# lqhl/rabitq-rs

Measured on AMD Instinct MI355X. Metric: queries/sec at recall@10>=0.95, GIST-1M d=960, batch=1024, higher is better.
Workload: dtype u8

## Files before the change

### include/rbq.h

```cpp
#ifndef RBQ_H
#define RBQ_H

#include <stddef.h>
#include <stdint.h>

#ifdef __cplusplus
extern "C" {
#endif

#define RBQ_OK                   0
#define RBQ_DIMENSION_MISMATCH   1
#define RBQ_INVALID_CONFIG       2
#define RBQ_EMPTY_INDEX          3
#define RBQ_IO                   4
#define RBQ_INVALID_PERSISTENCE  5
#define RBQ_DEVICE               6

#define RBQ_METRIC_L2 0
#define RBQ_METRIC_IP 1
#define RBQ_ROTATOR_MATRIX 0
#define RBQ_ROTATOR_FHT_KAC 1
#define RBQ_ROTATOR_NONE 2

#define RBQ_BATCH 32

typedef struct rbq_index rbq_index;
typedef struct rbq_builder rbq_builder;

typedef struct {
    uint32_t dim;
    uint32_t padded_dim;
    uint8_t  metric;
    uint8_t  rotator;
    uint8_t  ex_bits;
    uint8_t  reserved;
    uint64_t n_vectors;
    uint64_t n_lists;
    const uint8_t* rotator_blob;
    uint64_t rotator_len;
} rbq_header;

typedef struct {
    const float*    centroid;
    uint64_t        n;
    const uint64_t* ids;
    const uint8_t*  batch_data;
    uint64_t        batch_len;
    const uint8_t*  ex_codes;
    const float*    f_add_ex;
    const float*    f_rescale_ex;
} rbq_list_view;

typedef struct {
    uint64_t estimated;
    uint64_t skipped_by_lower_bound;
    uint64_t extended_evaluations;
} rbq_diag;

int rbq_index_create(const rbq_header* hdr, const rbq_list_view* lists,
                     int n_devices, const int* devices, rbq_index** out);

int rbq_index_load_rbq1(const void* bytes, size_t len,
                        int n_devices, const int* devices, rbq_index** out);

int rbq_index_build_device(const rbq_header* hdr, const float* centroids, const float* d_data, const uint32_t* d_assign,
                           uint64_t n, float t_const, int device, rbq_index** out);

#define RBQ_RESCALE_CONST   0
#define RBQ_RESCALE_OPTIMAL 1
int rbq_index_build_device_ex(const rbq_header* hdr, const float* centroids, const float* d_data, const uint32_t* d_assign,
                              uint64_t n, int rescale, float t_const, int device, rbq_index** out);

int rbq_build_stream_begin(const rbq_header* hdr, const float* centroids, const uint32_t* list_sizes, float t_const,
                           int device, rbq_builder** out);
int rbq_build_stream_begin_ex(const rbq_header* hdr, const float* centroids, const uint32_t* list_sizes, int rescale,
                              float t_const, int device, rbq_builder** out);
int rbq_build_stream_push(rbq_builder* b, const float* vectors, const uint32_t* assign, uint64_t first_id, uint64_t count);
int rbq_build_stream_finish(rbq_builder* b, int n_devices, const int* devices, rbq_index** out);
void rbq_build_stream_abort(rbq_builder* b);

void rbq_index_destroy(rbq_index* idx);

uint64_t rbq_index_len(const rbq_index* idx);
uint64_t rbq_index_cluster_count(const rbq_index* idx);
uint32_t rbq_index_dim(const rbq_index* idx);
uint32_t rbq_index_padded_dim(const rbq_index* idx);
uint32_t rbq_index_device_count(const rbq_index* idx);

int rbq_search_batch(const rbq_index* idx, const float* queries, uint64_t nq,
                     uint32_t query_dim, uint32_t top_k, uint32_t nprobe,
                     const uint32_t* filter_words, uint64_t filter_nbits,
                     uint64_t* out_ids, float* out_scores, uint32_t* out_counts,
                     rbq_diag* diag);

int rbq_posting_scan_batch(const rbq_index* idx, const float* queries, uint64_t nq, uint32_t query_dim,
                           uint32_t top_k, const uint32_t* list_ids, const uint32_t* list_counts,
                           uint32_t max_lists, uint64_t* out_ids, float* out_scores, uint32_t* out_counts);



int rbq_search_batch_device(const rbq_index* idx, const float* d_queries, uint64_t nq,
                            uint32_t query_dim, uint32_t top_k, uint32_t nprobe,
                            const uint32_t* d_filter_words, uint64_t filter_nbits,
                            uint64_t* d_out_ids, float* d_out_scores,
                            uint32_t* d_out_counts, rbq_diag* d_diag,
                            void* hip_stream);

int rbq_release_stream(rbq_index* idx, void* hip_stream);

int rbq_index_fetch_embeddings(const rbq_index* idx, const uint64_t* ids, uint64_t n, float* out, uint8_t* found);
int rbq_index_fetch_embeddings_device(const rbq_index* idx, const uint64_t* d_ids, uint64_t n, float* d_out,
                                      uint8_t* d_found, void* hip_stream);

void* rbq_host_alloc(size_t bytes);
void rbq_host_free(void* p);

int rbq_index_set_rerank_vectors(rbq_index* idx, const float* vectors, uint64_t n);

#define RBQ_NUMERIC_NATIVE_AVX512 0
#define RBQ_NUMERIC_NATIVE_AVX2   1
#define RBQ_NUMERIC_PORTABLE      2
int rbq_index_set_numeric_variant(rbq_index* idx, int variant);
int rbq_index_numeric_variant(const rbq_index* idx);

void   rbq_profile_begin(rbq_index* idx);
void   rbq_profile_end(rbq_index* idx);
double rbq_profile_stage_ms(const rbq_index* idx, const char* stage, uint64_t* launches);
uint64_t rbq_profile_stage_samples(const rbq_index* idx, const char* stage, float* out, uint64_t cap);
uint64_t rbq_profile_scan_bytes(const rbq_index* idx);
int rbq_profile_counters(const rbq_index* idx, uint64_t* out, uint32_t n);
void rbq_profile_select_stages(rbq_index* idx, uint32_t mask);
void rbq_profile_set_sampling(rbq_index* idx, uint32_t every);
uint64_t rbq_debug_rank_fallbacks(const rbq_index* idx);
void rbq_debug_tie_log_stats(const rbq_index* idx, uint64_t* out4);
int rbq_debug_stage_resources(rbq_index* idx, uint64_t nq, uint32_t top_k, uint32_t nprobe, uint32_t* out);
uint64_t rbq_debug_bounce_copies(void);
uint64_t rbq_debug_head_exact_evaluations(const rbq_index* idx);
uint64_t rbq_debug_head_exact_guard_trips(const rbq_index* idx);
uint64_t rbq_debug_heap_restarts(const rbq_index* idx);
int rbq_debug_copy_index(rbq_index* idx, const char* name, void* dst, uint64_t bytes);
int rbq_debug_best_rescale(const float* o_abs, uint64_t n, uint32_t dim, uint32_t ex_bits, int device, double* out_t);
int rbq_debug_copy_workspace(rbq_index* idx, void* hip_stream, const char* name, void* dst, uint64_t bytes);
int rbq_debug_set_option(rbq_index* idx, const char* name, int value);

int rbq_process_defaults(void);
const char* rbq_strerror(int code);
int rbq_last_error_detail(char* buf, size_t n);

uint32_t rbq_abi_version(void);

#ifdef __cplusplus
}
#endif

#include "rbq_bf.h"
#include "rbq_kmeans.h"
#include "rbq_persist.h"

#endif
```

### rabitq-rs_amd/csrc/device/api.hpp

```cpp
#pragma once
#include <hip/hip_runtime.h>

#include <algorithm>
#include <atomic>
#include <chrono>
#include <condition_variable>
#include <deque>
#include <functional>
#include <cmath>
#include <cstdio>
#include <cstdlib>
#include <cstring>
#include <map>
#include <memory>
#include <mutex>
#include <new>
#include <string>
#include <thread>
#include <vector>

#include "rbq.h"
#include "launch.hpp"
#include "../host/rbq_host_logic.hpp"

// ... 123 lines not shown
        if (e == hipSuccess) events.push_back(*ev);
        return e;
    }
};

template <class Job, int kThreads>
struct WorkerPool {
    std::thread th[kThreads];
    std::mutex mu;
    std::condition_variable cv;
    std::deque<Job> jobs;
    std::atomic<uint32_t> pending{0};
    bool stop = false;
    void run() {
        for (;;) {
            Job job;
            {
                std::unique_lock<std::mutex> lk(mu);
                cv.wait(lk, [this] { return stop || !jobs.empty(); });
                if (jobs.empty()) return;
                job = std::move(jobs.front());
                jobs.pop_front();
            }
            job();
            pending.fetch_sub(1, std::memory_order_release);
            (void)spin_until([this] { return pending.load(std::memory_order_acquire) != 0; }, std::chrono::microseconds(100));
        }
    }
    bool start() {
        try {
            for (auto& t : th) t = std::thread([this] { run(); });
        } catch (...) {
            shutdown();
            return false;
        }
        return true;
    }
    void post(Job j) {
        pending.fetch_add(1, std::memory_order_release);
        { std::lock_guard<std::mutex> lk(mu); jobs.push_back(std::move(j)); }
        cv.notify_one();
    }
    void shutdown() {
        { std::lock_guard<std::mutex> lk(mu); stop = true; }
        cv.notify_all();
        for (auto& t : th) if (t.joinable()) t.join();
    }
};

struct StageJob {
    void* dst = nullptr;
    const void* src = nullptr;
    size_t bytes = 0;
    std::atomic<int>* done = nullptr;
    void operator()() const {
        std::memcpy(dst, src, bytes);
        done->store(1, std::memory_order_release);
    }
};
using StagePool = WorkerPool<StageJob, 3>;

using ReplicaPool = WorkerPool<std::function<void()>, 2>;

struct Workspace {
    hipStream_t stream = nullptr;
    DevBuf queries, rot, lut, consts, scores, probe, wl, nstream, nvec, out_pack, filter, rot_hi, rot_lo, dead_skipped, heap_ws, key_window, audit_dead, tie_log, head_ub;
    DevBuf ms_sl, ms_lists;
    DevBuf mr_pool;
    PinBuf h_in, h_out;
    hipEvent_t done = nullptr;
    uint64_t call_nq = 0;
    bool latency_first = false;
    Workspace() = default;
    Workspace(const Workspace&) = delete;
    ~Workspace() {
        if (done) (void)hipEventDestroy(done);
        if (stream) (void)hipStreamDestroy(stream);
    }
};

struct StageProf {
    std::vector<std::pair<hipEvent_t, hipEvent_t>> ev;
    double ms = 0;
    uint64_t launches = 0;
    std::vector<float> samples;
};
struct EventPool {
    std::vector<std::pair<hipEvent_t, hipEvent_t>> free_pairs;
    bool take(std::pair<hipEvent_t, hipEvent_t>& p) {
        if (!free_pairs.empty()) { p = free_pairs.back(); free_pairs.pop_back(); return true; }
        if (hipEventCreateWithFlags(&p.first, hipEventDisableSystemFence) != hipSuccess) return false;
        if (hipEventCreateWithFlags(&p.second, hipEventDisableSystemFence) != hipSuccess) { (void)hipEventDestroy(p.first); return false; }
        return true;
    }
    void give(const std::pair<hipEvent_t, hipEvent_t>& p) { free_pairs.push_back(p); }
    void destroy() {
        for (auto& e : free_pairs) { (void)hipEventDestroy(e.first); (void)hipEventDestroy(e.second); }
        free_pairs.clear();
    }
};

struct Arr {
    void* p = nullptr;
    size_t bytes = 0;
};

struct Geometry {
    uint32_t dim = 0, D = 0, Dc = 0;
    uint8_t metric = 0, rotator = 0, ex_bits = 0;
    uint32_t trunc = 0;
    float fac = 1.0f;
};
inline Geometry geometry_of(const rbq_header& h) {
    Geometry g;
    g.dim = h.dim; g.D = h.padded_dim; g.Dc = (h.padded_dim + 63u) / 64u * 64u;
    g.metric = h.metric; g.rotator = h.rotator; g.ex_bits = h.ex_bits;
    uint32_t lg = 0;
    for (uint32_t x = h.dim; x >>= 1;) ++lg;
    g.trunc = 1u << lg;
    g.fac = 1.0f / std::sqrt((float)g.trunc);
    return g;
}

template <class Ws>
PrepParams prep_params(const Geometry& g, const Arr& rot_blob, Ws& w, const float* queries, uint64_t nq) {
    PrepParams p;
    p.queries = queries; p.nq = (uint32_t)nq; p.dim = g.dim; p.D = g.D; p.Dc = g.Dc; p.rotator = (int)g.rotator;
    p.rot_blob = (const uint8_t*)rot_blob.p; p.trunc = g.trunc; p.fac = g.fac; p.ex_bits = g.ex_bits;
    p.rot = (float*)w.rot.p; p.lut = (uint8_t*)w.lut.p; p.consts = (QueryConsts*)w.consts.p;
    p.rot_hi = nullptr; p.rot_lo = nullptr; p.wg_prep = false;
    return p;
}

inline int scan_wave_default() {
    static const int v = [] { const char* e = std::getenv("RBQ_SCAN_WAVE"); return e && *e ? std::atoi(e) : 2; }();
    return v;
}

struct Options {
    uint32_t numeric_variant = 0;
    uint32_t host_lanes = 0, host_subbatch = 0, host_trace = 0;
    int rank_ksplit = 1;
    bool host_zero_copy = true;
    bool host_stage_helpers = true;
    bool no_block_bound = false, f32_rank = false, wg_prep = false, exact_heap = false, force_rank_fallback = false, exact_rank = false;
    bool head_exact = true;
    bool lazy_filter = true;
    bool lazy_fault_inject = false;
    SlackMul slack;
    int slack_term = 0;
    bool ub_tap = false;
    bool lazy_audit = false;
    bool lazy_select = true;
    uint32_t tie_log_cap = 0;
    bool tie_log = true;
    int latency_path = 1;
    int rank_tile = 0;
    uint32_t stage_mask = 0xf;
    int scan_wave = scan_wave_default();
    bool profile_counters = true;
    uint64_t save_chunk = 0;
    uint64_t fetch_chunk = 0;
    uint64_t mstg_chunk = 0;
    uint64_t mstg_search_budget = 0;
    int set(const char* name, int value);
};

struct Replica : Geometry {
    int device = 0;
    uint64_t n_vectors = 0, n_lists = 0, n_blocks = 0;
    Arr rot_blob, centroids, blocks, ids, ex, fadd_ex, fres_ex, list_gb0, list_n, prof, bsum, cnorm2, fallbacks, cent_hi, cent_lo, raw,
        bsumx, lsum;
    Arr* arrays[18] = {&rot_blob, &centroids, &blocks, &ids, &ex, &fadd_ex, &fres_ex, &list_gb0, &list_n, &prof, &bsum, &cnorm2,
                       &fallbacks, &cent_hi, &cent_lo, &raw, &bsumx, &lsum};
    Arr delta, vl;
    Arr rnorm;
    bool has_rnorm = false, tc_some = false;
    float tc_value = 0.0f;
    bool has_recon = false;
    std::mutex fetch_mu;
    Arr fmap_ids, fmap_slots;
    bool fmap_ready = false;
    Arr ms_hi, ms_lo, ms_nc;
    bool ms_ready = false;
    uint32_t ms_bad = 0;
    Arr mr_slot_map, mr_blk_list;
    bool mr_ready = false;
    float cnorm2_max = 0.0f;
    uint64_t n_raw = 0;
    bool raw_borrowed = false;
    bool rerank = false;
    Options opt;
    std::unique_ptr<StagePool> stagers;
    bool stagers_failed = false;
    std::vector<uint32_t> h_list_n;
    std::vector<uint64_t> nblk_desc_prefix;
    std::mutex mu;
    std::vector<Workspace*> pool;
    std::map<hipStream_t, Workspace*> stream_ws;
    bool profiling = false;
    uint32_t prof_mask = 0xf;
    uint32_t prof_every = 1;
    uint32_t prof_seq[4] = {0, 0, 0, 0};
    StageProf stage_prof[4];
    EventPool ev_pool;
    uint64_t prof_counters[kProfSlots] = {0, 0, 0, 0, 0, 0, 0, 0};
    Replica() = default;
    Replica(const Replica&) = delete;
};

int alloc_arr(Arr& a, size_t bytes);
int upload_arr(Arr& a, const void* src, size_t bytes);
void free_replica(Replica* ix);
struct ReplicaOwner {
    Replica* ix;
    ~ReplicaOwner() { if (ix) free_replica(ix); }
    Replica* release() { Replica* r = ix; ix = nullptr; return r; }
};
int validate_header(const rbq_header* h, bool brute_force = false);
int resolve_devices(int n_devices, const int* devices, std::vector<int>& out);
Replica* new_replica(const rbq_header* hdr, int dev);
int finish_replica(Replica* ix, const std::vector<uint32_t>& ln);
int wrap_and_replicate(Replica* first, const std::vector<int>& devs, rbq_index** out);
int build_device_pairs(const rbq_header* hdr, const float* centroids, const float* d_data, const uint32_t* d_assign,
                       const uint32_t* d_vec, uint64_t n, int rescale, float t_const, int dev, rbq_index** out);

Workspace* take_ws(Replica* ix);
void give_ws(Replica* ix, Workspace* w);
Workspace* stream_workspace(Replica* ix, hipStream_t s);
int check_query_args(const rbq_index* h, uint32_t query_dim);
Replica* replica_of_pointer(rbq_index* h, const void* dptr);
struct ProfScope {
    Replica* ix; int stage; hipStream_t s; std::pair<hipEvent_t, hipEvent_t> ev{nullptr, nullptr};
    bool on = false, ext = false;
    ProfScope(Replica* ix_, int st, hipStream_t s_, bool ext_ = false) : ix(ix_), stage(st), s(s_), ext(ext_) {
        if (ix->profiling && !stage_probes() && ((ix->prof_mask >> st) & 1u)) {
            {
                std::lock_guard<std::mutex> g(ix->mu);
                if (ix->prof_seq[st]++ % ix->prof_every == 0) on = ix->ev_pool.take(ev);
            }
            if (on && !ext) (void)hipEventRecord(ev.first, s);
        }
    }
    hipEvent_t start() const { return on && ext ? ev.first : nullptr; }
    hipEvent_t stop() const { return on && ext ? ev.second : nullptr; }
    ~ProfScope() {
        if (on) {
            if (!ext) (void)hipEventRecord(ev.second, s);
            std::lock_guard<std::mutex> g(ix->mu);
            ix->stage_prof[stage].ev.push_back(ev);
        }
    }
};
int scan_stage(Replica* ix, Workspace* w, uint64_t nq, uint32_t probe_stride, uint32_t top_k, uint64_t wl_stride,
               const uint32_t* d_filter, uint64_t filter_nbits, uint64_t* d_ids, float* d_scores, uint32_t* d_counts,
               rbq_diag* d_diag, bool mstg, const uint32_t* d_dead_skipped, hipStream_t stream, const uint64_t* d_slot_ids = nullptr);

}

struct rbq_index {
    std::vector<rbq_api::Replica*> reps;
    int debug_replica = 0;
    std::mutex worker_mu;
    std::vector<std::unique_ptr<rbq_api::ReplicaPool>> workers;
};

#pragma GCC visibility pop
```

### rabitq-rs_amd/csrc/device/api_index.hip

```cpp
#include "api.hpp"

using namespace rbq_api;

extern "C" int rbq_process_defaults(void) {
    return RBQ_OK;
}

namespace rbq_api {
int alloc_arr(Arr& a, size_t bytes) {
    HIP_TRY(hipMalloc(&a.p, bytes ? bytes : 16));
    a.bytes = bytes;
    return RBQ_OK;
}
int upload_arr(Arr& a, const void* src, size_t bytes) {
    int rc = alloc_arr(a, bytes);
    if (rc) return rc;
    if (bytes) HIP_TRY(hipMemcpy(a.p, src, bytes, hipMemcpyHostToDevice));
    return RBQ_OK;
}

void free_replica(Replica* ix) {
    if (!ix) return;
    if (ix->stagers) ix->stagers->shutdown();
    DeviceGuard g(ix->device);
    (void)hipDeviceSynchronize();
    for (Arr* a : ix->arrays)
        if (a->p && !(a == &ix->raw && ix->raw_borrowed)) (void)hipFree(a->p);
    for (Arr* a : {&ix->delta, &ix->vl, &ix->rnorm, &ix->fmap_ids, &ix->fmap_slots, &ix->ms_hi, &ix->ms_lo, &ix->ms_nc,
                   &ix->mr_slot_map, &ix->mr_blk_list})
        if (a->p) (void)hipFree(a->p);
    for (Workspace* w : ix->pool) delete w;
    for (auto& kv : ix->stream_ws) delete kv.second;
    for (auto& sp : ix->stage_prof)
        for (auto& e : sp.ev) { (void)hipEventDestroy(e.first); (void)hipEventDestroy(e.second); }
    ix->ev_pool.destroy();
    delete ix;
}

int validate_header(const rbq_header* h, bool brute_force) {
    if (!h) return fail(RBQ_INVALID_CONFIG, "null header");
    if (h->dim == 0) return fail(RBQ_INVALID_CONFIG, "dimension must be positive");
    if (h->padded_dim < h->dim) return fail(RBQ_INVALID_CONFIG, "padded_dim must be >= dim");
    if (h->metric > 1) return fail(RBQ_INVALID_CONFIG, "unknown metric tag");
    if (h->rotator > (brute_force ? RBQ_ROTATOR_FHT_KAC : RBQ_ROTATOR_NONE)) return fail(RBQ_INVALID_CONFIG, "unknown rotator type tag");
    if (h->ex_bits != 0 && h->ex_bits != 2 && h->ex_bits != 6)
        return fail(RBQ_INVALID_CONFIG, "Unsupported ex_bits: only 0 (1-bit total), 2 (3-bit total), and 6 (7-bit total) are supported");
    if (h->padded_dim % 16 != 0) return fail(RBQ_INVALID_CONFIG, "Dimension must be multiple of 16 for SIMD");
    if (h->padded_dim > 2048)
        return fail(RBQ_INVALID_CONFIG, "padded_dim > 2048 (high-accuracy i32 LUT mode) is not supported");
    if (h->rotator_len != 0 && !h->rotator_blob) return fail(RBQ_INVALID_CONFIG, "null rotator blob");
    if (h->rotator == RBQ_ROTATOR_NONE) {
        if (h->padded_dim != h->dim) return fail(RBQ_INVALID_CONFIG, "rotator NONE requires padded_dim == dim");
        if (h->rotator_len != 0) return fail(RBQ_INVALID_CONFIG, "rotator NONE takes no rotator blob");
    } else if (h->rotator == RBQ_ROTATOR_FHT_KAC) {
        if (h->padded_dim % 64 != 0) return fail(RBQ_INVALID_CONFIG, "FHT rotator requires dimension to be multiple of 64");
        if (h->rotator_len != (uint64_t)4 * h->padded_dim / 8) return fail(RBQ_INVALID_PERSISTENCE, "FHT rotator flip bits length mismatch");
    } else {
        if (h->rotator_len != (uint64_t)h->padded_dim * h->padded_dim * 4) return fail(RBQ_INVALID_PERSISTENCE, "rotator matrix length mismatch");
    }
    if (brute_force) return RBQ_OK;
    if (h->n_lists == 0) return fail(RBQ_INVALID_CONFIG, "nlist must be positive");
    if (h->n_lists > 0xffffffffull) return fail(RBQ_INVALID_CONFIG, "too many lists");
    return RBQ_OK;
}

int resolve_devices(int n_devices, const int* devices, std::vector<int>& out) {
    if (n_devices < 1 || n_devices > 16) return fail(RBQ_INVALID_CONFIG, "n_devices must be in 1..16");
    int count = 0;
    HIP_TRY(hipGetDeviceCount(&count));
    out.clear();
    for (int i = 0; i < n_devices; ++i) {
        int d = 0;
        if (devices) d = devices[i];
        else if (n_devices == 1) HIP_TRY(hipGetDevice(&d));
        else d = i;
        if (d < 0 || d >= count) return fail(RBQ_INVALID_CONFIG, "no such device: " + std::to_string(d));
        out.push_back(d);
    }
    return RBQ_OK;
}

Replica* new_replica(const rbq_header* hdr, int dev) {
    Replica* ix = new Replica();
    static_cast<Geometry&>(*ix) = geometry_of(*hdr);
    ix->device = dev;
    ix->n_lists = hdr->n_lists;
    return ix;
}

int finish_replica(Replica* ix, const std::vector<uint32_t>& ln) {
    const uint32_t nlist = (uint32_t)ix->n_lists, D = ix->D;
    ix->h_list_n = ln;
    {
        std::vector<uint64_t> nblk(nlist);
        for (uint32_t c = 0; c < nlist; ++c) nblk[c] = (ln[c] + 31u) / 32u;
        std::sort(nblk.begin(), nblk.end(), std::greater<uint64_t>());
        ix->nblk_desc_prefix.assign((size_t)nlist + 1, 0);
        for (uint32_t c = 0; c < nlist; ++c) ix->nblk_desc_prefix[c + 1] = ix->nblk_desc_prefix[c] + nblk[c];
    }
    int rc;
    if ((rc = alloc_arr(ix->cnorm2, (size_t)nlist * 4))) return rc;
    if ((rc = alloc_arr(ix->cent_hi, (size_t)nlist * D * 2))) return rc;
    if ((rc = alloc_arr(ix->cent_lo, (size_t)nlist * D * 2))) return rc;
    HIP_TRY(launch_centroid_arrays((const float*)ix->centroids.p, nlist, D, (float*)ix->cnorm2.p, (uint16_t*)ix->cent_hi.p,
                                   (uint16_t*)ix->cent_lo.p, 0));
    std::vector<float> cn(nlist);
    HIP_TRY(hipMemcpy(cn.data(), ix->cnorm2.p, (size_t)nlist * 4, hipMemcpyDeviceToHost));
    double mx = 0;
    for (float v : cn) if (std::isfinite(v)) mx = std::max(mx, (double)v);
    ix->cnorm2_max = (float)(mx * 1.000001);
    if ((rc = alloc_arr(ix->lsum, (size_t)nlist * sizeof(BlockSummary)))) return rc;
    if ((rc = alloc_arr(ix->bsumx, ix->n_blocks * sizeof(BlockSummaryEx)))) return rc;
    HIP_TRY(launch_list_summaries((const uint8_t*)ix->blocks.p, (const uint8_t*)ix->ex.p, (const float*)ix->fadd_ex.p,
                                  (const float*)ix->fres_ex.p, (const float*)ix->centroids.p, (const BlockSummary*)ix->bsum.p,
                                  (const uint32_t*)ix->list_gb0.p, (const uint32_t*)ix->list_n.p, nlist, D, ix->Dc, ix->ex_bits,
                                  (BlockSummaryEx*)ix->bsumx.p, (BlockSummary*)ix->lsum.p, 0));
    if ((rc = alloc_arr(ix->fallbacks, 32))) return rc;
    HIP_TRY(hipMemset(ix->fallbacks.p, 0, 32));
    if ((rc = alloc_arr(ix->prof, (size_t)kProfStripes * kProfSlots * 8))) return rc;
    HIP_TRY(hipMemset(ix->prof.p, 0, (size_t)kProfStripes * kProfSlots * 8));
    const char* e = std::getenv("RBQ_EXACT_RANK");
    ix->opt.exact_rank = e && e[0] == '1';
    const char* f = std::getenv("RBQ_FORCE_RANK_FALLBACK");
    ix->opt.force_rank_fallback = f && f[0] == '1';
    const char* lz = std::getenv("RBQ_LAZY_SELECT");
    ix->opt.lazy_select = !(lz && lz[0] == '0');
    return RBQ_OK;
}

int Options::set(const char* name, int v) {
    const auto is = [name](const char* n) { return !std::strcmp(name, n); };
    if (is("block_bound")) no_block_bound = v == 0;
    else if (is("exact_rank")) exact_rank = v != 0;
    else if (is("exact_heap")) exact_heap = v != 0;
    else if (is("lazy_select")) lazy_select = v != 0;
    else if (is("rank_tile")) rank_tile = v;
    else if (is("latency_path")) latency_path = v;
    else if (is("tie_log")) tie_log = v != 0;
    else if (is("tie_log_cap")) tie_log_cap = v > 0 ? (uint32_t)v : 0u;
    else if (is("stage_mask")) stage_mask = (uint32_t)v & 0xfu;
    else if (is("scan_wave")) scan_wave = v < 0 ? scan_wave_default() : (v > 2 ? 2 : v);
    else if (is("profile_counters")) profile_counters = v != 0;
    else if (is("f32_rank")) f32_rank = v != 0;
    else if (is("wg_prep")) wg_prep = v != 0;
    else if (is("force_rank_fallback")) force_rank_fallback = v != 0;
    else if (is("host_lanes")) host_lanes = v > 0 ? (uint32_t)v : 0u;
    else if (is("host_subbatch")) host_subbatch = v > 0 ? (uint32_t)v : 0u;
    else if (is("host_trace")) host_trace = v != 0;
    else if (is("lazy_fault_inject")) lazy_fault_inject = v != 0;
    else if (is("lazy_audit")) lazy_audit = v != 0;
    else if (is("ub_tap")) ub_tap = v != 0;
    else if (is("save_chunk")) save_chunk = v > 0 ? (uint64_t)v : 0u;
    else if (is("fetch_chunk")) fetch_chunk = v > 0 ? (uint64_t)v : 0u;
    else if (is("mstg_chunk")) mstg_chunk = v > 0 ? (uint64_t)v : 0u;
    else if (is("mstg_search_budget")) mstg_search_budget = v > 0 ? (uint64_t)v : 0u;
    else if (is("slack_term")) slack_term = v;
    else if (is("slack_milli")) {
        float* f[6] = {&slack.ge, &slack.eip, &slack.est, &slack.lb, &slack.et, &slack.dist};
        if (slack_term < 0 || slack_term > 5) return fail(RBQ_INVALID_CONFIG, "slack_term is 0..5");
        *f[slack_term] = (float)v * 1e-3f;
    }
    else if (is("head_exact")) head_exact = v != 0;
    else if (is("lazy_filter")) lazy_filter = v != 0;
    else if (is("host_zero_copy")) host_zero_copy = v != 0;
    else if (is("rank_ksplit")) rank_ksplit = v < 0 ? 0 : v;
    else if (is("host_stage_helpers")) host_stage_helpers = v != 0;
    else return fail(RBQ_INVALID_CONFIG, std::string("unknown option ") + name);
    return RBQ_OK;
}
}

namespace rbq_api {
namespace {
void free_index(rbq_index* h) {
    if (!h) return;
    for (auto& w : h->workers) w->shutdown();
    for (Replica* r : h->reps) free_replica(r);
    delete h;
}

std::atomic<uint64_t> g_bounce_copies{0};
hipError_t copy_cross_device(void* dst, int ddev, const void* src, int sdev, size_t bytes) {
    if (!bytes) return hipSuccess;
    const char* fnp = std::getenv("RBQ_FORCE_NO_PEER");
    const bool no_peer = fnp && fnp[0] == '1';
    hipError_t e = hipSuccess;
    if (!no_peer) {
        if (ddev == sdev) return hipMemcpy(dst, src, bytes, hipMemcpyDeviceToDevice);
        int can = 0;
        if (hipDeviceCanAccessPeer(&can, ddev, sdev) == hipSuccess && can) {
            const hipError_t pe = hipDeviceEnablePeerAccess(sdev, 0);
            if (pe != hipSuccess) (void)hipGetLastError();
        } else {
            (void)hipGetLastError();
        }
        e = hipMemcpyPeer(dst, ddev, src, sdev, bytes);
        if (e == hipSuccess) return e;
        (void)hipGetLastError();
    }
    g_bounce_copies.fetch_add(1, std::memory_order_relaxed);
    const size_t CH = (size_t)64 << 20;
    void* bounce = nullptr;
    e = hipHostMalloc(&bounce, std::min(bytes, CH), hipHostMallocPortable);
    if (e != hipSuccess) return e;
    for (size_t off = 0; off < bytes && e == hipSuccess; off += CH) {
        const size_t n = std::min(CH, bytes - off);
        e = hipSetDevice(sdev);
        if (e == hipSuccess) e = hipMemcpy(bounce, (const uint8_t*)src + off, n, hipMemcpyDeviceToHost);
        if (e == hipSuccess) e = hipSetDevice(ddev);
        if (e == hipSuccess) e = hipMemcpy((uint8_t*)dst + off, bounce, n, hipMemcpyHostToDevice);
    }
    (void)hipSetDevice(ddev);
    (void)hipHostFree(bounce);
    return e;
}

int clone_replica(const Replica* src, int dev, Replica** out) {
    DeviceGuard g(dev);
    if (!g.ok) return fail(RBQ_DEVICE, "hipSetDevice failed");
    Replica* ix = new Replica();
    static_cast<Geometry&>(*ix) = *src;
    ix->device = dev;
    ix->n_vectors = src->n_vectors; ix->n_lists = src->n_lists; ix->n_blocks = src->n_blocks;
    ix->cnorm2_max = src->cnorm2_max; ix->h_list_n = src->h_list_n; ix->nblk_desc_prefix = src->nblk_desc_prefix;
    ix->opt = src->opt;
    for (size_t i = 0; i < sizeof(ix->arrays) / sizeof(ix->arrays[0]); ++i) {
        const Arr* s = src->arrays[i];
        Arr* d = ix->arrays[i];
        if (!s->p || s == &src->raw) continue;
        hipError_t e = hipMalloc(&d->p, s->bytes ? s->bytes : 16);
        if (e == hipSuccess && s->bytes) e = copy_cross_device(d->p, dev, s->p, src->device, s->bytes);
        if (e != hipSuccess) { free_replica(ix); return fail(RBQ_DEVICE, std::string("replicating the index: ") + hipGetErrorString(e)); }
        d->bytes = s->bytes;
    }
    hipError_t e = hipMemset(ix->fallbacks.p, 0, 32);
    if (e == hipSuccess) e = hipMemset(ix->prof.p, 0, (size_t)kProfStripes * kProfSlots * 8);
    if (e != hipSuccess) { free_replica(ix); return fail(RBQ_DEVICE, hipGetErrorString(e)); }
    *out = ix;
    return RBQ_OK;
}
}

int wrap_and_replicate(Replica* first, const std::vector<int>& devs, rbq_index** out) {
    rbq_index* h = new rbq_index();
    h->reps.push_back(first);
    for (size_t i = 1; i < devs.size(); ++i) {
        Replica* r = nullptr;
        int rc = clone_replica(first, devs[i], &r);
        if (rc) { free_index(h); return rc; }
        h->reps.push_back(r);
    }
    *out = h;
    return RBQ_OK;
}

namespace {
int create_from_sources(const rbq_header* hdr, const std::vector<ListSrc>& lists, int dev, Replica** out) {
    DeviceGuard g(dev);
    if (!g.ok) return fail(RBQ_DEVICE, "hipSetDevice failed");
    ReplicaOwner own{new_replica(hdr, dev)};
    Replica* ix = own.ix;
    Scratch cl;
    const uint32_t D = ix->D, Dc = ix->Dc, nlist = (uint32_t)ix->n_lists, exbits = ix->ex_bits;
    const size_t ref_stride = (size_t)D * 4 + 384, dev_stride = (size_t)Dc * 4 + 384, exb = (size_t)D * exbits / 8;
    const size_t exd = ex_bytes_dev(D, exbits);
    std::vector<uint32_t> gb0(nlist), ln(nlist);
    uint64_t nblocks = 0, nvec = 0;
    bool recon = true;
    for (uint32_t c = 0; c < nlist; ++c)
        if (lists[c].n && (!lists[c].delta || !lists[c].vl)) recon = false;
    for (uint32_t c = 0; c < nlist; ++c) {
        const ListSrc& L = lists[c];
        if (L.n > 0xffffffffull) return fail(RBQ_INVALID_CONFIG, "list too large");
        gb0[c] = (uint32_t)nblocks; ln[c] = (uint32_t)L.n;
        nblocks += (L.n + 31) / 32; nvec += L.n;
        if (nblocks * 32 > 0xffffffffull) return fail(RBQ_INVALID_CONFIG, "index too large for 32-bit vector slots");
    }
    ix->n_blocks = nblocks; ix->n_vectors = nvec;
    const uint64_t nslots = nblocks * 32;
    int rc;
    if ((rc = upload_arr(ix->rot_blob, hdr->rotator_blob, hdr->rotator_len))) return rc;
    if ((rc = upload_arr(ix->list_gb0, gb0.data(), (size_t)nlist * 4))) return rc;
    if ((rc = upload_arr(ix->list_n, ln.data(), (size_t)nlist * 4))) return rc;
    {
        std::vector<float> cent((size_t)nlist * D);
        for (uint32_t c = 0; c < nlist; ++c) std::memcpy(&cent[(size_t)c * D], lists[c].centroid, (size_t)D * 4);
        if ((rc = upload_arr(ix->centroids, cent.data(), cent.size() * 4))) return rc;
    }
    if ((rc = alloc_arr(ix->blocks, nblocks * dev_stride))) return rc;
    if ((rc = alloc_arr(ix->ids, nslots * 8))) return rc;
    if ((rc = alloc_arr(ix->ex, exd ? nslots * exd + 256 : 0))) return rc;
    if ((rc = alloc_arr(ix->fadd_ex, exbits ? nslots * 4 : 0))) return rc;
    if ((rc = alloc_arr(ix->fres_ex, exbits ? nslots * 4 : 0))) return rc;
    if ((rc = alloc_arr(ix->bsum, nblocks * sizeof(BlockSummary)))) return rc;
    if (recon) {
        if ((rc = alloc_arr(ix->delta, nslots * 4))) return rc;
        if ((rc = alloc_arr(ix->vl, nslots * 4))) return rc;
    }

    const size_t per_block = ref_stride + 32 * (exb + 24) + 12 + 64;
    uint64_t chunk_blocks = std::max<uint64_t>(1, ((size_t)64 << 20) / per_block);
    chunk_blocks = std::min<uint64_t>(chunk_blocks, std::max<uint64_t>(nblocks, 1));
    const size_t cap = align_up(chunk_blocks * ref_stride, 16) + align_up(chunk_blocks * 32 * exb, 16) + chunk_blocks * 32 * 24 +
                       chunk_blocks * 12 + 256;
    uint8_t* pin[2] = {nullptr, nullptr};
    uint8_t* dst[2] = {nullptr, nullptr};
    hipEvent_t ev[2] = {nullptr, nullptr};
    HIP_TRY(cl.make_stream());
    for (int i = 0; i < 2; ++i) {
        HIP_TRY(cl.alloc_pinned(&pin[i], cap));
        HIP_TRY(cl.alloc(&dst[i], cap));
        HIP_TRY(cl.event(&ev[i]));
    }
    uint32_t c = 0;
    uint64_t lb = 0;
    uint64_t b0 = 0;
    int turn = 0;
    while (b0 < nblocks) {
        const uint64_t nb = std::min<uint64_t>(chunk_blocks, nblocks - b0);
        const int i = turn & 1;
        if (turn >= 2) HIP_TRY(hipEventSynchronize(ev[i]));
        uint8_t* base = pin[i];
        const size_t o_recs = 0, o_ex = align_up(nb * ref_stride, 16);
        const size_t o_ids = o_ex + align_up(nb * 32 * exb, 16), o_fadd = o_ids + nb * 32 * 8, o_fres = o_fadd + nb * 32 * 4,
                     o_dl = o_fres + nb * 32 * 4, o_vl = o_dl + nb * 32 * 4, o_d0 = o_vl + nb * 32 * 4, o_nv = o_d0 + nb * 8,
                     total = o_nv + nb * 4;
        uint64_t* dense0 = reinterpret_cast<uint64_t*>(base + o_d0);
        uint32_t* nvb = reinterpret_cast<uint32_t*>(base + o_nv);
        uint64_t filled = 0, dense = 0;
        while (filled < nb) {
            while (c < nlist && lb >= ((uint64_t)ln[c] + 31) / 32) { ++c; lb = 0; }
            const ListSrc& L = lists[c];
            const uint64_t lnb = ((uint64_t)ln[c] + 31) / 32, take = std::min<uint64_t>(lnb - lb, nb - filled);
            const uint64_t v0 = lb * 32, v1 = std::min<uint64_t>(L.n, (lb + take) * 32), nv = v1 - v0;
            std::memcpy(base + o_recs + filled * ref_stride, L.batch_data + lb * ref_stride, take * ref_stride);
            if (nv) std::memcpy(base + o_ids + dense * 8, L.ids + v0 * 8, nv * 8);
            if (exbits && nv) {
                if (L.ex_stride == exb) std::memcpy(base + o_ex + dense * exb, L.ex + v0 * exb, nv * exb);
                else for (uint64_t v = 0; v < nv; ++v) std::memcpy(base + o_ex + (dense + v) * exb, L.ex + (v0 + v) * L.ex_stride, exb);
                std::memcpy(base + o_fadd + dense * 4, L.fadd + v0 * 4, nv * 4);
                std::memcpy(base + o_fres + dense * 4, L.fres + v0 * 4, nv * 4);
            }
            if (recon && nv) {
                std::memcpy(base + o_dl + dense * 4, L.delta + v0 * 4, nv * 4);
                std::memcpy(base + o_vl + dense * 4, L.vl + v0 * 4, nv * 4);
            }
            for (uint64_t b = 0; b < take; ++b) {
                dense0[filled + b] = dense + b * 32;
                nvb[filled + b] = (uint32_t)std::min<uint64_t>(32, L.n - (lb + b) * 32);
            }
            filled += take; dense += nv; lb += take;
        }
        uint8_t* d = dst[i];
        HIP_TRY(hipMemcpyAsync(d, base, total, hipMemcpyHostToDevice, cl.stream));
        const uint64_t* d_d0 = reinterpret_cast<const uint64_t*>(d + o_d0);
        const uint32_t* d_nv = reinterpret_cast<const uint32_t*>(d + o_nv);
        uint8_t* oblocks = (uint8_t*)ix->blocks.p + b0 * dev_stride;
        HIP_TRY(launch_relayout_blocks(d + o_recs, (uint32_t)nb, D, Dc, oblocks, cl.stream));
        HIP_TRY(launch_block_summary(oblocks, d_nv, (uint32_t)nb, Dc, (BlockSummary*)ix->bsum.p + b0, cl.stream));
        HIP_TRY(launch_spread_u64(reinterpret_cast<const uint64_t*>(d + o_ids), d_d0, d_nv, (uint32_t)nb, ~0ull,
                                  (uint64_t*)ix->ids.p + b0 * 32, cl.stream));
        if (exbits) {
            HIP_TRY(launch_relayout_ex(d + o_ex, d_d0, d_nv, (uint32_t)nb, D, exbits, (uint8_t*)ix->ex.p + b0 * 32 * exd, cl.stream));
            HIP_TRY(launch_spread_f32(reinterpret_cast<const float*>(d + o_fadd), d_d0, d_nv, (uint32_t)nb, 0.0f,
                                      (float*)ix->fadd_ex.p + b0 * 32, cl.stream));
            HIP_TRY(launch_spread_f32(reinterpret_cast<const float*>(d + o_fres), d_d0, d_nv, (uint32_t)nb, 0.0f,
                                      (float*)ix->fres_ex.p + b0 * 32, cl.stream));
        }
        if (recon) {
            HIP_TRY(launch_spread_f32(reinterpret_cast<const float*>(d + o_dl), d_d0, d_nv, (uint32_t)nb, 0.0f,
                                      (float*)ix->delta.p + b0 * 32, cl.stream));
            HIP_TRY(launch_spread_f32(reinterpret_cast<const float*>(d + o_vl), d_d0, d_nv, (uint32_t)nb, 0.0f,
                                      (float*)ix->vl.p + b0 * 32, cl.stream));
        }
        HIP_TRY(hipEventRecord(ev[i], cl.stream));
        b0 += nb;
        ++turn;
    }
    if (exd) HIP_TRY(hipMemsetAsync((uint8_t*)ix->ex.p + nslots * exd, 0, 256, cl.stream));
    HIP_TRY(hipStreamSynchronize(cl.stream));
    if ((rc = finish_replica(ix, ln))) return rc;
    HIP_TRY(hipDeviceSynchronize());
    ix->has_recon = recon;
    *out = own.release();
    return RBQ_OK;
}

int create_impl(const rbq_header* hdr, const rbq_list_view* lists, const float* const* delta, const float* const* vl, int n_devices,
// ... 137 lines not shown
                if (e != hipSuccess) rc = fail(RBQ_DEVICE, std::string("attaching the rerank vectors: ") + hipGetErrorString(e));
            }
        }
        if (rc != RBQ_OK) {
            const std::string keep = g_err;
            for (size_t r = 0; r < R; ++r)
                if (fresh[r].p && !borrowed[r]) { DeviceGuard g(h->reps[r]->device); (void)hipFree(fresh[r].p); }
            return fail(rc, keep);
        }
    }
    for (size_t r = 0; r < R; ++r) {
        Replica* ix = h->reps[r];
        DeviceGuard g(ix->device);
        if (!g.ok) return fail(RBQ_DEVICE, "hipSetDevice failed");
        HIP_TRY(hipDeviceSynchronize());
        if (ix->raw.p && !ix->raw_borrowed) (void)hipFree(ix->raw.p);
        ix->raw = Arr(); ix->n_raw = 0; ix->rerank = false; ix->raw_borrowed = false;
        if (!attach) continue;
        ix->raw = fresh[r]; ix->raw_borrowed = borrowed[r] != 0;
        ix->n_raw = n; ix->rerank = true;
    }
    return RBQ_OK;
    RBQ_GUARD_END
}

void* rbq_host_alloc(size_t bytes) {
    void* p = nullptr;
    if (hipHostMalloc(&p, bytes ? bytes : 16, hipHostMallocPortable) != hipSuccess) { (void)hipGetLastError(); return nullptr; }
    return p;
}
void rbq_host_free(void* p) { if (p) (void)hipHostFree(p); }

void rbq_profile_begin(rbq_index* h) {
    if (!h) return;
    for (Replica* ix : h->reps) {
        DeviceGuard g(ix->device);
        std::lock_guard<std::mutex> lk(ix->mu);
        for (auto& sp : ix->stage_prof) {
            for (auto& e : sp.ev) ix->ev_pool.give(e);
            sp.ev.clear(); sp.ms = 0; sp.launches = 0; sp.samples.clear();
        }
        for (auto& c : ix->prof_counters) c = 0;
        (void)hipMemset(ix->prof.p, 0, (size_t)kProfStripes * kProfSlots * 8);
        ix->profiling = true;
    }
}
void rbq_profile_end(rbq_index* h) {
    if (!h) return;
    for (Replica* ix : h->reps) {
        DeviceGuard g(ix->device);
        (void)hipDeviceSynchronize();
        std::lock_guard<std::mutex> lk(ix->mu);
        ix->profiling = false;
        std::vector<unsigned long long> c((size_t)kProfStripes * kProfSlots, 0ull);
        (void)hipMemcpy(c.data(), ix->prof.p, c.size() * 8, hipMemcpyDeviceToHost);
        for (int i = 0; i < kProfSlots; ++i) {
            ix->prof_counters[i] = 0;
            for (uint32_t st = 0; st < kProfStripes; ++st) ix->prof_counters[i] += c[(size_t)st * kProfSlots + i];
        }
        for (auto& sp : ix->stage_prof) {
            for (auto& e : sp.ev) {
                float ms = 0;
                if (hipEventElapsedTime(&ms, e.first, e.second) == hipSuccess) { sp.ms += ms; sp.launches++; sp.samples.push_back(ms); }
                ix->ev_pool.give(e);
            }
            sp.ev.clear();
        }
    }
}
double rbq_profile_stage_ms(const rbq_index* h, const char* stage, uint64_t* launches) {
    if (!h || h->reps.empty() || !stage) return -1;
    int s = !std::strcmp(stage, "prep") ? 0 : !std::strcmp(stage, "rank") ? 1 : !std::strcmp(stage, "select") ? 2 : !std::strcmp(stage, "scan") ? 3 : -1;
    if (s < 0) return -1;
    double ms = 0; uint64_t n = 0;
    for (const Replica* ix : h->reps) { ms += ix->stage_prof[s].ms; n += ix->stage_prof[s].launches; }
    if (launches) *launches = n;
    return n ? ms / (double)n : 0.0;
}
uint64_t rbq_profile_stage_samples(const rbq_index* h, const char* stage, float* out, uint64_t cap) {
    if (!h || h->reps.empty() || !stage) return 0;
    int s = !std::strcmp(stage, "prep") ? 0 : !std::strcmp(stage, "rank") ? 1 : !std::strcmp(stage, "select") ? 2 : !std::strcmp(stage, "scan") ? 3 : -1;
    if (s < 0) return 0;
    uint64_t n = 0;
    for (const Replica* ix : h->reps)
        for (float v : ix->stage_prof[s].samples) { if (out && n < cap) out[n] = v; ++n; }
    return n;
}
uint64_t rbq_profile_scan_bytes(const rbq_index* h) {
    if (!h || h->reps.empty()) return 0;
    uint64_t v = 0;
    for (const Replica* ix : h->reps) v += ix->prof_counters[kProfVectorsProbed];
    return v * (uint64_t)(h->reps[0]->D / 8 + 12);
}
int rbq_profile_counters(const rbq_index* h, uint64_t* out, uint32_t n) {
    if (!h || h->reps.empty() || !out) return RBQ_INVALID_CONFIG;
    for (uint32_t i = 0; i < n; ++i) {
        out[i] = 0;
        if (i < (uint32_t)kProfSlots) for (const Replica* ix : h->reps) out[i] += ix->prof_counters[i];
    }
    return RBQ_OK;
}
void rbq_profile_select_stages(rbq_index* h, uint32_t mask) { if (h) for (Replica* ix : h->reps) ix->prof_mask = mask & 0xfu; }
void rbq_profile_set_sampling(rbq_index* h, uint32_t every) { if (h) for (Replica* ix : h->reps) ix->prof_every = every ? every : 1u; }

int rbq_index_set_numeric_variant(rbq_index* h, int variant) {
    g_err.clear();
    if (!h || h->reps.empty()) return fail(RBQ_INVALID_CONFIG, "null index");
    if (variant != RBQ_NUMERIC_NATIVE_AVX512 && variant != RBQ_NUMERIC_NATIVE_AVX2 && variant != RBQ_NUMERIC_PORTABLE)
        return fail(RBQ_INVALID_CONFIG, "numeric variant " + std::to_string(variant) +
                                            " is not one of 0 (native_avx512), 1 (native_avx2), 2 (portable)");
    static_assert(RBQ_NUMERIC_NATIVE_AVX512 == kVarAvx512 && RBQ_NUMERIC_NATIVE_AVX2 == kVarAvx2 && RBQ_NUMERIC_PORTABLE == kVarPortable,
                  "the ABI values are the kernels' variant numbers");
    for (Replica* ix : h->reps) ix->opt.numeric_variant = (uint32_t)variant;
    return RBQ_OK;
}
int rbq_index_numeric_variant(const rbq_index* h) {
    if (!h || h->reps.empty()) return -1;
    return (int)h->reps[0]->opt.numeric_variant;
}

int rbq_debug_set_option(rbq_index* h, const char* name, int value) {
    if (!h || h->reps.empty() || !name) return RBQ_INVALID_CONFIG;
    if (!std::strcmp(name, "numeric_variant")) return rbq_index_set_numeric_variant(h, value);
    if (!std::strcmp(name, "debug_replica")) {
        if (value < 0 || (size_t)value >= h->reps.size()) return fail(RBQ_INVALID_CONFIG, "no such replica");
        h->debug_replica = value;
        return RBQ_OK;
    }
    for (Replica* ix : h->reps) {
        int rc;
        if (!std::strcmp(name, "rerank")) {
            if (value && !ix->raw.p) return fail(RBQ_INVALID_CONFIG, "no raw vectors attached (rbq_index_set_rerank_vectors)");
            ix->rerank = value != 0;
        } else if ((rc = ix->opt.set(name, value))) {
            return rc;
        }
    }
    return RBQ_OK;
}
static uint64_t read_counter(const rbq_index* h, int slot) {
    if (!h) return 0;
    uint64_t tot = 0;
    for (const Replica* ix : h->reps) {
        unsigned int v = 0;
        DeviceGuard g(ix->device);
        (void)hipDeviceSynchronize();
        (void)hipMemcpy(&v, (const unsigned int*)ix->fallbacks.p + slot, 4, hipMemcpyDeviceToHost);
        tot += v;
    }
    return tot;
}
uint64_t rbq_debug_rank_fallbacks(const rbq_index* h) { return read_counter(h, 0); }
void rbq_debug_tie_log_stats(const rbq_index* h, uint64_t* out4) { if (out4) for (int i = 0; i < 4; ++i) out4[i] = read_counter(h, 4 + i); }
uint64_t rbq_debug_head_exact_guard_trips(const rbq_index* h) { return read_counter(h, 2); }
uint64_t rbq_debug_head_exact_evaluations(const rbq_index* h) { return read_counter(h, 3); }


uint64_t rbq_debug_bounce_copies(void) { return g_bounce_copies.load(std::memory_order_relaxed); }
uint64_t rbq_debug_heap_restarts(const rbq_index* h) { return read_counter(h, 1); }


int rbq_debug_copy_workspace(rbq_index* h, void* hip_stream, const char* name, void* dst, uint64_t bytes) {
    g_err.clear();
    RBQ_GUARD_BEGIN
    if (!h || h->reps.empty() || !name || !dst) return RBQ_INVALID_CONFIG;
    Replica* ix = h->reps[h->debug_replica];
    Workspace* w = nullptr;
    {
        std::lock_guard<std::mutex> lk(ix->mu);
        auto it = ix->stream_ws.find((hipStream_t)hip_stream);
        if (it != ix->stream_ws.end()) w = it->second;
    }
    if (!w) return fail(RBQ_INVALID_CONFIG, "no workspace for this stream");
    static const std::pair<const char*, DevBuf Workspace::*> kBufs[] = {
        {"rot", &Workspace::rot}, {"lut", &Workspace::lut}, {"consts", &Workspace::consts}, {"scores", &Workspace::scores},
        {"probe", &Workspace::probe}, {"nstream", &Workspace::nstream}, {"wl", &Workspace::wl}, {"nvec", &Workspace::nvec},
        {"dead_skipped", &Workspace::dead_skipped}, {"audit_dead", &Workspace::audit_dead}, {"head_ub", &Workspace::head_ub},
        {"rot_hi", &Workspace::rot_hi}, {"rot_lo", &Workspace::rot_lo}};
    DevBuf* b = nullptr;
    for (const auto& kb : kBufs) if (!std::strcmp(name, kb.first)) b = &(w->*kb.second);
    if (!b || !b->p || bytes > b->cap) return fail(RBQ_INVALID_CONFIG, "unknown buffer or size");
    DeviceGuard g(ix->device);
    HIP_TRY(hipMemcpy(dst, b->p, bytes, hipMemcpyDeviceToHost));
    return RBQ_OK;
    RBQ_GUARD_END
}

int rbq_debug_copy_index(rbq_index* h, const char* name, void* dst, uint64_t bytes) {
    g_err.clear();
    RBQ_GUARD_BEGIN
    if (!h || h->reps.empty() || !name || !dst) return RBQ_INVALID_CONFIG;
    Replica* ix = h->reps[h->debug_replica];
    const size_t stride = (size_t)ix->Dc * 4 + 384, exd = ex_bytes_dev(ix->D, ix->ex_bits), slots = ix->n_blocks * 32;
    const void* p = nullptr;
    size_t have = 0;
    if (!std::strcmp(name, "blocks")) { p = ix->blocks.p; have = ix->n_blocks * stride; }
    else if (!std::strcmp(name, "ids")) { p = ix->ids.p; have = slots * 8; }
    else if (!std::strcmp(name, "ex")) { p = ix->ex.p; have = slots * exd; }
    else if (!std::strcmp(name, "fadd_ex")) { p = ix->fadd_ex.p; have = ix->ex_bits ? slots * 4 : 0; }
    else if (!std::strcmp(name, "fres_ex")) { p = ix->fres_ex.p; have = ix->ex_bits ? slots * 4 : 0; }
    else if (!std::strcmp(name, "bsum")) { p = ix->bsum.p; have = ix->n_blocks * sizeof(BlockSummary); }
    else if (!std::strcmp(name, "lsum")) { p = ix->lsum.p; have = ix->n_lists * sizeof(BlockSummary); }
    else if (!std::strcmp(name, "bsumx")) { p = ix->bsumx.p; have = ix->n_blocks * sizeof(BlockSummaryEx); }
    else if (!std::strcmp(name, "centroids")) { p = ix->centroids.p; have = ix->n_lists * ix->D * 4; }
    else if (!std::strcmp(name, "list_gb0")) { p = ix->list_gb0.p; have = ix->n_lists * 4; }
    else if (!std::strcmp(name, "list_n")) { p = ix->list_n.p; have = ix->n_lists * 4; }
    else if (!std::strcmp(name, "cent_hi")) { p = ix->cent_hi.p; have = ix->n_lists * ix->D * 2; }
    else if (!std::strcmp(name, "cent_lo")) { p = ix->cent_lo.p; have = ix->n_lists * ix->D * 2; }
    else if (!std::strcmp(name, "cnorm2")) { p = ix->cnorm2.p; have = ix->n_lists * 4; }
    else if (!std::strcmp(name, "delta") || !std::strcmp(name, "vl")) {
        ix = h->reps[0];
        p = name[0] == 'd' ? ix->delta.p : ix->vl.p; have = ix->has_recon ? ix->n_blocks * 32 * 4 : 0;
    }
    else if (!std::strcmp(name, "rnorm")) {
        ix = h->reps[0];
        p = ix->rnorm.p; have = ix->has_rnorm ? ix->n_blocks * 32 * 4 : 0;
    }
    if (!p || bytes != have) return fail(RBQ_INVALID_CONFIG, "unknown array or size (have " + std::to_string(have) + " bytes)");
    DeviceGuard g(ix->device);
    HIP_TRY(hipMemcpy(dst, p, bytes, hipMemcpyDeviceToHost));
    return RBQ_OK;
    RBQ_GUARD_END
}
}
```

### rabitq-rs_amd/csrc/device/api_search.hip

```cpp
#include "api.hpp"

using namespace rbq_api;

namespace rbq_api {
namespace {
constexpr uint64_t kScanWaveMinQueries = 128;
constexpr uint64_t kHostWaveMinQueries = 4096;
constexpr uint64_t kLatMaxQueries = 4;
constexpr uint64_t kLatMaxBytes = 96ull << 20;
constexpr uint64_t kSplitKMaxCallQueries = 256;
constexpr uint64_t kPrepWgMaxQueries = 512;
constexpr uint64_t kZeroCopyMinQueries = 5;


bool is_pinned_host_range(const void* p, size_t bytes) {
    if (!p) return false;
    hipPointerAttribute_t a, b;
    if (hipPointerGetAttributes(&a, p) != hipSuccess) { (void)hipGetLastError(); return false; }
    if (a.type != hipMemoryTypeHost) return false;
    if (bytes <= 1) return true;
    const uint8_t* last = (const uint8_t*)p + bytes - 1;
    if (hipPointerGetAttributes(&b, last) != hipSuccess) { (void)hipGetLastError(); return false; }
    if (b.type != hipMemoryTypeHost) return false;
    if (a.devicePointer && b.devicePointer && (const uint8_t*)b.devicePointer - (const uint8_t*)a.devicePointer != (ptrdiff_t)(bytes - 1)) return false;
// ... 42 lines not shown
    if (hipPointerGetAttributes(&a, dptr) == hipSuccess) {
        for (Replica* r : h->reps) if (r->device == a.device) return r;
    } else {
        (void)hipGetLastError();
    }
    return h->reps[0];
}

int scan_stage(Replica* ix, Workspace* w, uint64_t nq, uint32_t probe_stride, uint32_t top_k, uint64_t wl_stride,
               const uint32_t* d_filter, uint64_t filter_nbits, uint64_t* d_ids, float* d_scores, uint32_t* d_counts,
               rbq_diag* d_diag, bool mstg, const uint32_t* d_dead_skipped, hipStream_t stream, const uint64_t* d_slot_ids) {
    ProfScope ps(ix, 3, stream, true);
    ScanParams P;
    P.blocks = (const uint8_t*)ix->blocks.p; P.ids = d_slot_ids ? d_slot_ids : (const uint64_t*)ix->ids.p; P.ex_codes = (const uint8_t*)ix->ex.p;
    P.f_add_ex = (const float*)ix->fadd_ex.p; P.f_rescale_ex = (const float*)ix->fres_ex.p;
    P.lut = (const uint8_t*)w->lut.p; P.rot = (const float*)w->rot.p; P.consts = (const QueryConsts*)w->consts.p;
    P.probe = (const ProbeInfo*)w->probe.p; P.wl = (const StreamItem*)w->wl.p; P.nstream = (const uint32_t*)w->nstream.p;
    P.filter = d_filter; P.filter_nbits = filter_nbits; P.wl_stride = wl_stride;
    P.out_ids = d_ids; P.out_scores = d_scores; P.out_counts = d_counts; P.diag = (unsigned long long*)d_diag;
    P.D = ix->D; P.Dc = ix->Dc; P.nprobe = probe_stride; P.top_k = top_k; P.metric = ix->metric;
    P.ex_bits = mstg ? 0u : ix->ex_bits;
    P.no_block_bound = ix->opt.no_block_bound ? 1u : 0u;
    P.exact_heap = ix->opt.exact_heap ? 1u : 0u;
    P.heap_restarts = (unsigned int*)ix->fallbacks.p + 1;
    P.tie_stats = (unsigned int*)ix->fallbacks.p + 4;
    P.mstg = mstg ? 1u : 0u;
    P.prof = (ix->profiling && ix->opt.profile_counters) ? (unsigned long long*)ix->prof.p : nullptr;
    P.dead_skipped = d_dead_skipped;
    P.numeric_variant = ix->opt.numeric_variant;
    P.wave_kernel = (ix->opt.scan_wave == 1 || (ix->opt.scan_wave == 2 && nq >= kScanWaveMinQueries && !ix->opt.no_block_bound && !w->latency_first)) ? 1u : 0u;
    P.tie_log = nullptr; P.tie_log_cap = 0;
    if (ix->opt.tie_log && !P.wave_kernel && !d_diag && !mstg && top_k >= 1 && top_k <= kTopKRegMax && !ix->opt.exact_heap && !stage_probes()) {
        const uint32_t cap = ix->opt.tie_log_cap ? ix->opt.tie_log_cap : (top_k < 64u ? 2048u : 8192u);
        if ((uint64_t)nq * cap * 12u <= (1ull << 30)) {
            if (w->tie_log.ensure((size_t)nq * cap * 12u) == RBQ_OK) { P.tie_log = (uint32_t*)w->tie_log.p; P.tie_log_cap = cap; }
            else { (void)hipGetLastError(); g_err.clear(); }
        }
    }
    P.heap_ws = nullptr;
    if (top_k > kTopKMax || scan_lds_bytes(ix->Dc, ix->D, P.ex_bits, top_k) > kLdsPerWorkgroupMax) {
        int rc = w->heap_ws.ensure((size_t)nq * 2 * ((size_t)top_k + 1) * 4);
        if (rc) return rc;
        P.heap_ws = (uint32_t*)w->heap_ws.p;
    }
    HIP_TRY(launch_scan(P, (uint32_t)nq, ix->device, stream, ps.start(), ps.stop()));
    return RBQ_OK;
}

namespace {
int search_device(Replica* ix, Workspace* w, const float* d_queries, uint64_t nq, uint32_t top_k, uint32_t nprobe_in,
                  const uint32_t* d_filter, uint64_t filter_nbits, uint64_t* d_ids, float* d_scores, uint32_t* d_counts,
                  rbq_diag* d_diag, hipStream_t stream) {
    const uint32_t D = ix->D, Dc = ix->Dc;
    const uint32_t nlist = (uint32_t)ix->n_lists;
    uint32_t nprobe = nprobe_in < 1 ? 1 : nprobe_in;
    if (nprobe > nlist) nprobe = nlist;
    const bool big_nprobe = nprobe > kNprobeMax;
    const bool heap_in_global = top_k > kTopKMax || scan_lds_bytes(Dc, D, ix->ex_bits, top_k) > kLdsPerWorkgroupMax;
    if (top_k > kTopKHardMax || (heap_in_global && (uint64_t)nq * ((uint64_t)top_k + 1) * 8 > (8ull << 30)))
        return fail(RBQ_INVALID_CONFIG, "top_k too large for one call (top_k <= 2^20 and nq * top_k * 8 bytes of heap workspace <= 8 GiB)");
    if (ix->rerank && top_k > 1024) return fail(RBQ_INVALID_CONFIG, "rerank supports top_k <= 1024");
    const uint64_t wl_stride = std::max<uint64_t>(ix->nblk_desc_prefix[nprobe], 1);

    int rc;
    if ((rc = w->rot.ensure(nq * D * 4))) return rc;
    if ((rc = w->lut.ensure(nq * (size_t)Dc * 4))) return rc;
    if ((rc = w->consts.ensure(nq * sizeof(QueryConsts)))) return rc;
    if ((rc = w->scores.ensure(nq * (size_t)nlist * 4))) return rc;
    if ((rc = w->probe.ensure(nq * (size_t)nprobe * sizeof(ProbeInfo)))) return rc;
    if ((rc = w->wl.ensure(nq * wl_stride * sizeof(StreamItem)))) return rc;
    if ((rc = w->nstream.ensure(nq * 4))) return rc;
    if ((rc = w->nvec.ensure(nq * 8))) return rc;
    if ((rc = w->dead_skipped.ensure(nq * 16))) return rc;
    const bool split_rank = !ix->opt.exact_rank && !ix->opt.f32_rank && D % 64 == 0;
    if (split_rank) {
        if ((rc = w->rot_hi.ensure(nq * D * 2))) return rc;
        if ((rc = w->rot_lo.ensure(nq * D * 2))) return rc;
    }
    unsigned long long* prof = (ix->profiling && ix->opt.profile_counters) ? (unsigned long long*)ix->prof.p : nullptr;
    const uint32_t smask = ix->opt.stage_mask;
    uint32_t ksplit = 1;
    if (ix->opt.rank_ksplit && ix->opt.latency_path && nq <= kPrepWgMaxQueries && (w->call_nq ? w->call_nq : nq) <= kSplitKMaxCallQueries && ix->rotator != 0 &&
        !ix->opt.wg_prep && D % 16 == 0 && split_rank && !ix->opt.exact_rank && !big_nprobe && smask == 0xfu) {
        const uint32_t T = ((uint64_t)((nlist + 127) / 128) * ((nq + 127) / 128) >= 192 && ix->opt.rank_tile != 64) || ix->opt.rank_tile == 128 ? 128u : 64u;
        const uint64_t tiles = (uint64_t)((nlist + T - 1) / T) * ((nq + T - 1) / T);
        ksplit = tiles >= 512 ? 1u : (tiles >= 256 ? 2u : 4u);
        while (ksplit > 1 && (D / 32) / ksplit < 6) ksplit >>= 1;
        if (ix->opt.rank_ksplit > 1) ksplit = (uint32_t)std::min(ix->opt.rank_ksplit, 4);
    }
    const bool lat_front = ix->opt.latency_path && nq <= kLatMaxQueries && ix->rotator != 0 && !ix->opt.wg_prep && !ix->opt.exact_rank && !big_nprobe &&
                           !ix->opt.f32_rank && (uint64_t)nlist * D * 4 * nq <= kLatMaxBytes && D % 16 == 0 && smask == 0xfu;
    if (lat_front) {
        ProfScope ps(ix, 0, stream);
        const PrepParams p = prep_params(*ix, ix->rot_blob, *w, d_queries, nq);
        RankParams r;
        r.metric = ix->metric; r.cent = (const float*)ix->centroids.p; r.nlist = nlist; r.D = D; r.nq = (uint32_t)nq;
        r.scores = (float*)w->scores.p;
        HIP_TRY(launch_lat_front(p, r, ix->device, stream));
    } else if (smask & 1u) {
        ProfScope ps(ix, 0, stream);
        PrepParams p = prep_params(*ix, ix->rot_blob, *w, d_queries, nq);
        p.rot_hi = split_rank ? (uint16_t*)w->rot_hi.p : nullptr; p.rot_lo = split_rank ? (uint16_t*)w->rot_lo.p : nullptr;
        p.wg_prep = ix->opt.wg_prep;
        if (ix->opt.latency_path && nq <= kPrepWgMaxQueries && ix->rotator != 0 && !ix->opt.wg_prep && D % 16 == 0) {
            RankParams r;
            r.metric = ix->metric; r.cent = nullptr; r.nlist = nlist; r.D = D; r.nq = (uint32_t)nq;
            r.scores = ksplit > 1 ? (float*)w->scores.p : nullptr; r.ksplit = ksplit;
            HIP_TRY(launch_lat_front(p, r, ix->device, stream));
        } else {
            HIP_TRY(launch_prep(p, ix->device, stream));
        }
    }
    RankParams rp;
    rp.metric = ix->metric; rp.rot = (const float*)w->rot.p; rp.rot_hi = (const uint16_t*)w->rot_hi.p; rp.rot_lo = (const uint16_t*)w->rot_lo.p;
    rp.cent = (const float*)ix->centroids.p; rp.cent_hi = (const uint16_t*)ix->cent_hi.p; rp.cent_lo = (const uint16_t*)ix->cent_lo.p;
    rp.consts = (const QueryConsts*)w->consts.p; rp.cnorm2 = (const float*)ix->cnorm2.p; rp.nq = (uint32_t)nq; rp.nlist = nlist; rp.D = D;
    rp.scores = (float*)w->scores.p; rp.split = split_rank; rp.ksplit = ksplit;
    rp.big = (uint64_t)((nlist + 127) / 128) * ((nq + 127) / 128) >= 192;
    rp.wide = ix->opt.rank_tile == 256 || (ix->opt.rank_tile == 0 && (uint64_t)((nlist + 255) / 256) * ((nq + 127) / 128) >= 2048);
    if (ix->opt.rank_tile == 64) rp.big = false;
    if (ix->opt.rank_tile == 128) rp.big = true;
    SelectParams sp;
    sp.scores = (float*)w->scores.p; sp.nq = (uint32_t)nq; sp.nlist = nlist; sp.nprobe = nprobe; sp.metric = ix->metric;
    sp.rot = (const float*)w->rot.p; sp.cent = (const float*)ix->centroids.p; sp.D = D; sp.consts = (const QueryConsts*)w->consts.p;
    sp.cnorm2_max = ix->cnorm2_max; sp.list_gb0 = (const uint32_t*)ix->list_gb0.p; sp.list_n = (const uint32_t*)ix->list_n.p;
    sp.probe = (ProbeInfo*)w->probe.p; sp.wl = (StreamItem*)w->wl.p; sp.wl_stride = wl_stride; sp.nstream = (uint32_t*)w->nstream.p;
    sp.nvec = (unsigned long long*)w->nvec.p; sp.prof_total = prof; sp.fallback_count = (unsigned int*)ix->fallbacks.p;
    sp.force_fallback = ix->opt.force_rank_fallback ? 1 : 0; sp.bsum = (const BlockSummary*)ix->bsum.p;
    sp.cnorm2 = (const float*)ix->cnorm2.p; sp.lsum = (const BlockSummary*)ix->lsum.p; sp.bsumx = (const BlockSummaryEx*)ix->bsumx.p;
    sp.dead_skipped = (uint32_t*)w->dead_skipped.p; sp.top_k = top_k; sp.ex_bits = ix->ex_bits;
    sp.slack = ix->opt.slack;
    sp.numeric_variant = ix->opt.numeric_variant;
    sp.audit_dead = nullptr;
    if (ix->opt.lazy_audit) {
        if ((rc = w->audit_dead.ensure(nq * (size_t)(kAuditCap + 1) * 4))) return rc;
        HIP_TRY(hipMemsetAsync(w->audit_dead.p, 0, nq * (size_t)(kAuditCap + 1) * 4, stream));
        sp.audit_dead = (uint32_t*)w->audit_dead.p;
    }
    sp.head_ub = nullptr;
    if (ix->opt.ub_tap) {
        if ((rc = w->head_ub.ensure(nq * (size_t)kHeadUbRow * 4))) return rc;
        HIP_TRY(hipMemsetAsync(w->head_ub.p, 0, nq * (size_t)kHeadUbRow * 4, stream));
        sp.head_ub = (uint32_t*)w->head_ub.p;
    }
    const bool lazy_with_filter = ix->opt.lazy_filter && ix->opt.head_exact && !d_diag;
    sp.lazy = (ix->opt.lazy_select && (!d_filter || lazy_with_filter) && !ix->opt.no_block_bound) ? 1 : 0;
    sp.filter = d_filter; sp.filter_nbits = filter_nbits; sp.ids = (const uint64_t*)ix->ids.p;
    sp.exact_members = d_diag ? 1 : 0;
    sp.fault_dead_all = ix->opt.lazy_fault_inject ? 1 : 0;
    sp.lut = (const uint8_t*)w->lut.p; sp.blocks = (const uint8_t*)ix->blocks.p; sp.ex_codes = (const uint8_t*)ix->ex.p;
    sp.f_add_ex = (const float*)ix->fadd_ex.p; sp.f_rescale_ex = (const float*)ix->fres_ex.p; sp.Dc = Dc;
    sp.head_exact = ix->opt.head_exact ? 1 : 0;
    sp.n_blocks = (uint32_t)ix->n_blocks;
    if (ix->opt.exact_rank || big_nprobe) {
        uint64_t* kw = nullptr;
        if (big_nprobe) {
            if ((rc = w->key_window.ensure((size_t)nq * select_exact_np2(nprobe) * 8))) return rc;
            kw = (uint64_t*)w->key_window.p;
        }
        if (smask & 2u) { ProfScope ps(ix, 1, stream); HIP_TRY(launch_rank_exact(rp, stream)); }
        if (smask & 4u) { ProfScope ps(ix, 2, stream); HIP_TRY(launch_select_exact(sp, ix->device, stream, kw)); }
    } else {
        if ((smask & 2u) && !lat_front) { ProfScope ps(ix, 1, stream); HIP_TRY(launch_rank_gemm(rp, ix->device, stream)); }
        if (smask & 4u) { ProfScope ps(ix, 2, stream); HIP_TRY(launch_select_mfma(sp, ix->device, stream)); }
    }
    if ((smask & 8u) && (rc = scan_stage(ix, w, nq, nprobe, top_k, wl_stride, d_filter, filter_nbits, d_ids, d_scores, d_counts, d_diag,
                         false, (ix->opt.exact_rank || big_nprobe) ? nullptr : (const uint32_t*)w->dead_skipped.p, stream)))
        return rc;
    if (ix->rerank && !stage_probes())
        HIP_TRY(launch_rerank(d_queries, (uint32_t)nq, ix->dim, (const float*)ix->raw.p, ix->n_raw, ix->metric, top_k, d_ids, d_scores,
                              d_counts, stream));
    return RBQ_OK;
}

int search_host(Replica* ix, const float* queries, uint64_t nq, uint32_t query_dim, uint32_t top_k, uint32_t nprobe,
                const uint32_t* filter_words, uint64_t filter_nbits, uint64_t* out_ids, float* out_scores, uint32_t* out_counts,
                rbq_diag* diag) {
    DeviceGuard g(ix->device);
    if (!g.ok) return fail(RBQ_DEVICE, "hipSetDevice failed");
    using clk = std::chrono::steady_clock;
    const bool trace = ix->opt.host_trace != 0;
    double t_attr = 0, t_ws = 0, t_stage = 0, t_enq = 0, t_wait = 0, t_out = 0;
    auto tick = [&](clk::time_point& t0, double& acc) { if (trace) { const auto t1 = clk::now(); acc += std::chrono::duration<double, std::micro>(t1 - t0).count(); t0 = t1; } };
    clk::time_point tp = clk::now();
    const std::vector<std::pair<uint64_t, uint64_t>> plan = rbq_host::subbatch_plan(nq, ix->opt.host_subbatch);
    const uint64_t nsub = plan.size();
    const uint32_t nlanes = (uint32_t)std::min<uint64_t>(nsub, ix->opt.host_lanes ? ix->opt.host_lanes : 6u);
    const bool in_pinned = is_pinned_host_range(queries, nq * query_dim * 4);
    bool out_pinned = !ix->rerank && is_pinned_host_range(out_ids, nq * top_k * 8) && is_pinned_host_range(out_scores, nq * top_k * 4) &&
                      is_pinned_host_range(out_counts, nq * 4) && (!diag || is_pinned_host_range(diag, nq * sizeof(rbq_diag)));
    uint64_t* c_ids = nullptr; float* c_scores = nullptr; uint32_t* c_counts = nullptr; rbq_diag* c_diag = nullptr;
    if (out_pinned) {
        if (hipHostGetDevicePointer((void**)&c_ids, out_ids, 0) != hipSuccess || hipHostGetDevicePointer((void**)&c_scores, out_scores, 0) != hipSuccess ||
            hipHostGetDevicePointer((void**)&c_counts, out_counts, 0) != hipSuccess ||
            (diag && hipHostGetDevicePointer((void**)&c_diag, diag, 0) != hipSuccess)) {
            (void)hipGetLastError();
            out_pinned = false;
        }
    }
    const bool zero_copy = ix->opt.host_zero_copy && nq >= kZeroCopyMinQueries && nq <= (in_pinned ? 1536u : 1024u);
    const float* c_queries = nullptr;
    if (zero_copy && in_pinned && hipHostGetDevicePointer((void**)&c_queries, const_cast<float*>(queries), 0) != hipSuccess) {
        (void)hipGetLastError();
        c_queries = nullptr;
    }
    tick(tp, t_attr);
    std::vector<Workspace*> lanes;
    struct Give { Replica* ix; std::vector<Workspace*>& l; bool drained = false;
                  ~Give() { for (Workspace* w : l) { if (!drained) (void)hipStreamSynchronize(w->stream); give_ws(ix, w); } } } give{ix, lanes};
    for (uint32_t i = 0; i < nlanes; ++i) {
        Workspace* w = take_ws(ix);
        if (!w) return fail(RBQ_DEVICE, "cannot create workspace stream");
        lanes.push_back(w);
    }
    tick(tp, t_ws);
    int rc;
    const uint32_t* d_filter = nullptr;
    if (filter_words) {
        const size_t fb = (size_t)((filter_nbits + 31) / 32) * 4;
        Workspace* w0 = lanes[0];
        if ((rc = w0->filter.ensure(fb ? fb : 4))) return rc;
        if (fb) HIP_TRY(hipMemcpyAsync(w0->filter.p, filter_words, fb, hipMemcpyHostToDevice, w0->stream));
        HIP_TRY(hipEventRecord(w0->done, w0->stream));
        for (uint32_t i = 1; i < nlanes; ++i) HIP_TRY(hipStreamWaitEvent(lanes[i]->stream, w0->done, 0));
        d_filter = (const uint32_t*)w0->filter.p;
    }
    auto deliver = [&](Workspace* w, uint64_t j) -> int {
        clk::time_point td = clk::now();
        HIP_TRY(hipEventSynchronize(w->done));
        tick(td, t_wait);
        if (out_pinned) return RBQ_OK;
        const uint64_t q0 = plan[j].first, n = plan[j].second;
        const OutPack op(n, top_k, diag != nullptr);
        const uint8_t* src = (const uint8_t*)w->h_out.p;
        std::memcpy(out_ids + q0 * top_k, src + op.o_ids, n * top_k * 8);
        std::memcpy(out_scores + q0 * top_k, src + op.o_scores, n * top_k * 4);
        std::memcpy(out_counts + q0, src + op.o_counts, n * 4);
        if (diag) std::memcpy(diag + q0, src + op.o_diag, n * sizeof(rbq_diag));
        tick(td, t_out);
        return RBQ_OK;
    };
    constexpr uint64_t kMaxHelped = 8;
    std::atomic<int> staged[kMaxHelped];
    uint64_t n_helped = 0;
    auto wait_staged = [&staged](uint64_t j) { spin_until([&] { return staged[j].load(std::memory_order_acquire) != 0; }); };
    struct WaitHelpers { decltype(wait_staged)& wait; uint64_t& n;
        ~WaitHelpers() { for (uint64_t j = 1; j <= n; ++j) wait(j); } } wait_helpers{wait_staged, n_helped};
    bool helpers = !in_pinned && ix->opt.host_stage_helpers && nsub >= 2 && nsub <= nlanes && nsub <= kMaxHelped && nq * query_dim * 4 >= (512u << 10);
    if (helpers) {
        std::lock_guard<std::mutex> lk(ix->mu);
        if (!ix->stagers && !ix->stagers_failed) {
            std::unique_ptr<StagePool> sh(new (std::nothrow) StagePool());
            if (sh && sh->start()) ix->stagers = std::move(sh);
            else ix->stagers_failed = true;
        }
        helpers = ix->stagers != nullptr;
    }
    if (helpers) {
        for (uint64_t j = 1; j < nsub; ++j) {
            Workspace* wj = lanes[j];
            if ((rc = wj->h_in.ensure(plan[j].second * query_dim * 4))) return rc;
            staged[j].store(0, std::memory_order_relaxed);
            ix->stagers->post(StageJob{wj->h_in.p, queries + plan[j].first * query_dim, (size_t)(plan[j].second * query_dim * 4), &staged[j]});
            n_helped = j;
        }
    }
    for (uint64_t j = 0; j < nsub; ++j) {
        Workspace* w = lanes[j % nlanes];
        if (j >= nlanes && (rc = deliver(w, j - nlanes))) return rc;
        const uint64_t q0 = plan[j].first, n = plan[j].second;
        const OutPack op(n, top_k, diag != nullptr);
        const bool staged_in_hbm = !(c_queries || (zero_copy && !in_pinned));
        if (staged_in_hbm && (rc = w->queries.ensure(n * query_dim * 4))) return rc;
        const float* src = queries + q0 * query_dim;
        tp = clk::now();
        const float* d_q = (const float*)w->queries.p;
        if (c_queries) {
            d_q = c_queries + q0 * query_dim;
        } else if (zero_copy && !in_pinned) {
            if (j >= 1 && j <= n_helped) {
                wait_staged(j);
            } else {
                if ((rc = w->h_in.ensure(n * query_dim * 4))) return rc;
                std::memcpy(w->h_in.p, src, n * query_dim * 4);
            }
            float* hp = nullptr;
            HIP_TRY(hipHostGetDevicePointer((void**)&hp, w->h_in.p, 0));
            d_q = hp;
        } else if (in_pinned) {
            HIP_TRY(hipMemcpyAsync(w->queries.p, src, n * query_dim * 4, hipMemcpyHostToDevice, w->stream));
        } else if (j >= 1 && j <= n_helped) {
            wait_staged(j);
            HIP_TRY(hipMemcpyAsync(w->queries.p, w->h_in.p, n * query_dim * 4, hipMemcpyHostToDevice, w->stream));
        } else {
            if ((rc = w->h_in.ensure(n * query_dim * 4))) return rc;
            const uint64_t piece = std::max<uint64_t>(64, (n + 3) / 4);
            for (uint64_t p0 = 0; p0 < n; p0 += piece) {
                const size_t off = p0 * query_dim * 4, len = std::min(piece, n - p0) * query_dim * 4;
                std::memcpy((uint8_t*)w->h_in.p + off, (const uint8_t*)src + off, len);
                HIP_TRY(hipMemcpyAsync((uint8_t*)w->queries.p + off, (const uint8_t*)w->h_in.p + off, len, hipMemcpyHostToDevice, w->stream));
            }
        }
        tick(tp, t_stage);
        uint64_t* k_ids; float* k_scores; uint32_t* k_counts; rbq_diag* k_diag;
        if (out_pinned) {
            k_ids = c_ids + q0 * top_k; k_scores = c_scores + q0 * top_k; k_counts = c_counts + q0; k_diag = diag ? c_diag + q0 : nullptr;
// ... 186 lines not shown
```

### rabitq-rs_amd/csrc/device/launch.hpp

```cpp
#pragma once
#include <atomic>
#include <string>

#include "types.hpp"

namespace rbq_host { struct HcResult; }

namespace rbq {

struct LdsAttrCache {
    std::atomic<size_t> set[16];
    LdsAttrCache() { for (auto& v : set) v.store(0, std::memory_order_relaxed); }
    hipError_t ensure(const void* fn, size_t lds, int device);
};

struct KernelProbe { const void* fn = nullptr; uint32_t grid_x = 0, grid_y = 0, grid_z = 0, block = 0; size_t dyn_lds = 0; };
struct StageProbes { KernelProbe k[4]; };
StageProbes*& stage_probes();
inline bool probe_stage(int stage, const void* fn, dim3 grid, uint32_t block, size_t lds) {
    StageProbes* p = stage_probes();
    if (!p) return false;
    p->k[stage].fn = fn; p->k[stage].grid_x = grid.x; p->k[stage].grid_y = grid.y; p->k[stage].grid_z = grid.z;
    p->k[stage].block = block; p->k[stage].dyn_lds = lds;
    return true;
}

struct PrepParams {
    const float* queries;
    uint32_t nq, dim, D, Dc;
    int rotator;
    const uint8_t* rot_blob;
    uint32_t trunc;
    float fac;
    uint32_t ex_bits;
    float* rot;
    uint8_t* lut;
    QueryConsts* consts;
    uint16_t *rot_hi, *rot_lo;
    bool wg_prep;
};
hipError_t launch_prep(const PrepParams& p, int device, hipStream_t s);

struct RankParams {
    int metric;
    const float* rot;
    const uint16_t *rot_hi, *rot_lo;
    const float* cent;
    const uint16_t *cent_hi, *cent_lo;
    const QueryConsts* consts;
    const float* cnorm2;
    uint32_t nq, nlist, D;
    float* scores;
    bool split;
    bool big;
    bool wide;
    uint32_t ksplit = 0;
};
hipError_t launch_rank_exact(const RankParams& p, hipStream_t s);
hipError_t launch_rank_gemm(const RankParams& p, int device, hipStream_t s);
hipError_t launch_lat_front(const PrepParams& p, const RankParams& r, int device, hipStream_t s);

constexpr uint32_t kAuditCap = 1023;
constexpr uint32_t kHeadUbRow = 2 + 8 + 3 * 256;
struct SelectParams {
    float* scores;
    uint32_t nq, nlist, nprobe;
    int metric;
    const float* rot;
    const float* cent;
    uint32_t D;
    const QueryConsts* consts;
    float cnorm2_max;
    const uint32_t *list_gb0, *list_n;
    ProbeInfo* probe;
    StreamItem* wl;
    uint64_t wl_stride;
    uint32_t* nstream;
    unsigned long long* nvec;
    unsigned long long* prof_total;
    unsigned int* fallback_count;
    int force_fallback;
    const BlockSummary* bsum;
    const float* cnorm2;
    const BlockSummary* lsum;
    const BlockSummaryEx* bsumx;
    uint32_t* dead_skipped;
    uint32_t top_k, ex_bits;
    int lazy;
    int exact_members;
    const uint8_t* lut;
    const uint8_t* blocks;
    const uint8_t* ex_codes;
    const float *f_add_ex, *f_rescale_ex;
    uint32_t Dc;
    uint32_t n_blocks;
    const uint32_t* filter;
    uint64_t filter_nbits;
    const uint64_t* ids;
    int head_exact;
    SlackMul slack;
    uint32_t* audit_dead;
    uint32_t* head_ub;
    uint32_t numeric_variant;
    int fault_dead_all;
};
uint32_t select_exact_np2(uint32_t nprobe);
hipError_t launch_select_exact(const SelectParams& p, int device, hipStream_t s, uint64_t* key_window);
hipError_t launch_select_mfma(const SelectParams& p, int device, hipStream_t s);

struct ProbesGivenParams {
    const uint32_t *list_ids, *list_counts;
    uint32_t max_lists, nq, nlist;
    int metric;
    const float* rot;
    const float* cent;
    uint32_t D;
    const uint32_t *list_gb0, *list_n;
    ProbeInfo* probe;
    StreamItem* wl;
    uint64_t wl_stride;
    uint32_t* nstream;
    const QueryConsts* consts;
    const BlockSummary* bsum;
    uint32_t numeric_variant;
};
hipError_t launch_probes_given(const ProbesGivenParams& p, hipStream_t s);

hipError_t launch_scan(const ScanParams& P, uint32_t nq, int device, hipStream_t s, hipEvent_t ev0, hipEvent_t ev1);
bool scanw_serves(const ScanParams& P);
hipError_t launch_scanw(const ScanParams& P, uint32_t nq, int device, hipStream_t s, hipEvent_t ev0, hipEvent_t ev1);

hipError_t launch_rotate_rows(const float* src, const uint32_t* map, uint32_t nrows, uint32_t dim, uint32_t D, int rotator,
                              const uint8_t* rot_blob, uint32_t trunc, float fac, float* rows, hipStream_t s);
hipError_t launch_encode(const EncodeParams& P, hipStream_t s);
hipError_t launch_rescale(const float* rows, const float* centroids, const uint32_t* block_list, const uint32_t* row_slot,
                          const uint32_t* slot_src, uint32_t nrows, uint32_t D, uint32_t ex_bits, bool raw_o, double* t,
                          hipStream_t s);
hipError_t launch_pack_ex(const uint8_t* raw, const uint32_t* slot_src, const uint32_t* row_slot, uint32_t nrows, uint32_t D,
                          uint32_t ex_bits, uint8_t* ex, hipStream_t s);
hipError_t launch_block_summary(const uint8_t* blocks, const uint32_t* block_nv, uint32_t nblocks, uint32_t Dc, BlockSummary* bsum,
                                hipStream_t s);
hipError_t launch_list_summaries(const uint8_t* blocks, const uint8_t* ex, const float* fadd_ex, const float* fres_ex, const float* cent,
                                 const BlockSummary* bsum, const uint32_t* list_gb0, const uint32_t* list_n, uint32_t nlist, uint32_t D,
                                 uint32_t Dc, uint32_t ex_bits, BlockSummaryEx* bsumx, BlockSummary* lsum, hipStream_t s);
hipError_t launch_count_assign(const uint32_t* assign, uint64_t n, uint32_t nlist, uint32_t* counts, uint32_t* err, hipStream_t s);
hipError_t launch_iota(uint32_t* x, uint64_t n, hipStream_t s);
hipError_t launch_scatter_slots(const uint32_t* sorted_list, const uint32_t* sorted_src, uint64_t n, const uint32_t* list_gb0,
                                const uint64_t* vstart, uint32_t* slot_src, hipStream_t s);
hipError_t sort_pairs_u32(void* tmp, size_t* tmp_bytes, const uint32_t* keys_in, uint32_t* keys_out, const uint32_t* vals_in,
                          uint32_t* vals_out, size_t n, unsigned bits, hipStream_t s);
hipError_t launch_chunk_first(const uint32_t* sorted_list, uint32_t n, uint32_t* chunk_first, hipStream_t s);
hipError_t launch_chunk_slots(const uint32_t* sorted_list, const uint32_t* sorted_src, uint32_t n, const uint32_t* list_gb0,
                              const uint32_t* list_cursor, const uint32_t* chunk_first, uint32_t* row_src, uint32_t* row_slot,
                              hipStream_t s);
hipError_t launch_chunk_advance(const uint32_t* sorted_list, uint32_t n, const uint32_t* chunk_first, uint32_t* list_cursor,
                                hipStream_t s);
hipError_t launch_relayout_blocks(const uint8_t* recs, uint32_t nb, uint32_t D, uint32_t Dc, uint8_t* blocks, hipStream_t s);
hipError_t launch_relayout_ex(const uint8_t* exsrc, const uint64_t* block_dense0, const uint32_t* block_nv,
                              uint32_t nb, uint32_t D, uint32_t ex_bits, uint8_t* ex, hipStream_t s);
hipError_t launch_spread_u64(const uint64_t* src, const uint64_t* block_dense0, const uint32_t* block_nv, uint32_t nb, uint64_t fill,
                             uint64_t* dst, hipStream_t s);
hipError_t launch_spread_f32(const float* src, const uint64_t* block_dense0, const uint32_t* block_nv, uint32_t nb, float fill,
                             float* dst, hipStream_t s);
hipError_t launch_centroid_arrays(const float* cent, uint32_t nlist, uint32_t D, float* cnorm2, uint16_t* hi, uint16_t* lo,
                                  hipStream_t s);
hipError_t launch_rerank(const float* queries, uint32_t nq, uint32_t dim, const float* raw, uint64_t n_raw, int metric,
                         uint32_t top_k, uint64_t* ids, float* scores, const uint32_t* counts, hipStream_t s);

struct BfDistParams {
    const float* rot;
    const QueryConsts* consts;
    uint32_t nq, D, ex_bits;
    uint64_t v0, nv;
    const uint8_t* bin;
    const uint8_t* ex;
    const float *f_add, *f_rescale, *f_add_ex, *f_rescale_ex;
    const uint32_t* filter;
    uint64_t filter_nbits;
    float* dist;
};
hipError_t launch_bf_dist(const BfDistParams& p, hipStream_t s);
struct BfSelectParams {
    const float* dist;
    uint32_t nq, top_k;
    uint64_t v0, nv;
    int metric;
    int first, last;
    bool lds_heap;
    float* heap_d;
    uint32_t* heap_s;
    uint32_t* heap_len;
    uint64_t* out_ids;
    float* out_scores;
    uint32_t* out_counts;
    unsigned long long* stats;
};
hipError_t launch_bf_select(const BfSelectParams& p, hipStream_t s);
constexpr uint32_t kBfLdsHeapMaxTopK = 8191;
hipError_t launch_bf_encode(const EncodeParams& P, hipStream_t s);
hipError_t launch_bf_pack_ex(const uint8_t* raw, uint64_t nrows, uint32_t D, uint32_t ex_bits, uint8_t* ex, hipStream_t s);

constexpr uint64_t kKmeansChunkBytes = 512ull << 20;
struct KMeansArgs {
    const float* data;
    uint64_t n;
    uint32_t dim;
    uint64_t k, niter, nredo, seed;
    int spherical;
    uint64_t mppc, dbs;
    int device;
    float* centroids;
    uint32_t* assignments;
    double* objective;
    uint64_t* stats;
};
int kmeans_device(const KMeansArgs& a, std::string& detail);

constexpr uint32_t kMstgMaxReplicas = 64;
struct ClosureArgs {
    const float* centroids;
    uint64_t k;
    uint32_t dim;
    const float* data;
    uint64_t n;
    float epsilon;
    uint32_t max_replicas;
    uint64_t max_chunk_rows;
    bool cent_on_device, data_on_device, out_on_device;
    uint32_t* out_lists;
    uint32_t* out_counts;
    uint32_t* tap_sl;
    uint32_t* tap_sl_n;
    uint64_t* fallbacks;
};
int closure_device(const ClosureArgs& a, int device, std::string& detail);
hipError_t launch_closure_expand(const uint32_t* lists, const uint32_t* counts, const uint32_t* off, uint64_t n, uint32_t max_replicas,
                                 uint32_t* pair_list, uint32_t* pair_vec, hipStream_t s);

struct HClusterArgs {
    const float* d_data;
    const float* h_data;
    uint64_t n;
    uint32_t dim;
    uint64_t max_size, k, niter;
    float balance_weight;
    uint64_t host_below;
    int device;
};
int hcluster_device(const HClusterArgs& a, rbq_host::HcResult& out, std::string& detail);

constexpr uint32_t kMsCap = 2048;
struct MstgSelectParams {
    const float* rot;
    uint32_t nq, D, k;
    uint32_t ef_search;
    float pruning_epsilon;
    const float* cent;
    const uint16_t *cent_hi, *cent_lo;
// ... 116 lines not shown
```

### rabitq-rs_amd/csrc/device/rank_mfma.hpp

```cpp
#pragma once
#include "kernels.hpp"

namespace rbq {

#ifndef RBQ_CANON_UNROLL
#define RBQ_CANON_UNROLL 4
#endif
typedef float f32x16 __attribute__((ext_vector_type(16)));

template <int METRIC, int TW>
__global__ __launch_bounds__(256) void k_rank_mfma(const float* __restrict__ rot, const float* __restrict__ cent,
                                                   const QueryConsts* __restrict__ consts,
                                                   const float* __restrict__ cnorm2, uint32_t nq, uint32_t nlist,
                                                   uint32_t D, float* __restrict__ scores) {
    constexpr int BM = 64 * TW, BN = 64 * TW, BK = 32, LD = BK + 1;
    __shared__ float As[BM][LD];
    __shared__ float Bs[BN][LD];
    const uint32_t tid = threadIdx.x, lane = tid & 63u, w = tid >> 6, wm = w >> 1, wn = w & 1u;
    const uint32_t q0 = blockIdx.y * BM, c0 = blockIdx.x * BN;
    f32x16 acc[TW][TW];
#pragma unroll
    for (int a = 0; a < TW; ++a)
#pragma unroll
        for (int b = 0; b < TW; ++b)
// ... 617 lines not shown
            uint4 xx[KG];
#pragma unroll
            for (int u = 0; u < KG; ++u) xx[u] = g0 + (uint32_t)u < G16 ? cp[(g0 + u) * 32] : make_uint4(0u, 0u, 0u, 0u);
#pragma unroll
            for (int u = 0; u < KG; ++u) {
                if (g0 + (uint32_t)u < G16) {
                    const uint8_t* lg = lutL + (g0 + u) * 512;
                    acc += hx_look8(xx[u].x, lg) + hx_look8(xx[u].y, lg + 128) + hx_look8(xx[u].z, lg + 256) + hx_look8(xx[u].w, lg + 384);
                }
            }
        }
        if (Dc & 64u) acc += hx_look8(ytail.x, lutL + G16 * 512) + hx_look8(ytail.y, lutL + G16 * 512 + 128);
        const float ip = epi_ip(qc.delta, (float)(acc & 0xffffu), qc.sum_vl, V == kVarPortable);
        const float tt = ip + qc.k1x;
        const float rs = f_rescale * tt;
        float est = f_add + g_add;
        const float e0 = est;
        est = est + rs;
        const float er = fminf(f_error * ge_lo, f_error * ge_hi);
        const float lb = est - er;
        bool ok = hx_tame(f_add) && hx_tame(f_rescale) && hx_tame(f_error) && hx_tame(ip) && hx_tame(rs) && hx_tame(e0) && hx_tame(est) &&
                  hx_tame(f_error * ge_lo) && hx_tame(f_error * ge_hi) && hx_tame(lb) && qc.amax <= 65535.0f;
        if (P.filter) {
            const uint32_t id32 = (uint32_t)P.ids[(size_t)(gb + b) * 32u + l32];
            ok = ok && ((uint64_t)id32 < P.filter_nbits) && ((P.filter[id32 >> 5] >> (id32 & 31u)) & 1u);
        }
        vEst[tid] = ok ? est : INFINITY;
        vLb[tid] = lb;
        vIp[tid] = ip;
    }
    __syncthreads();
    float* res = reinterpret_cast<float*>(part);
    if (tid == 0) res[0] = INFINITY;
    if (ex_bits == 0) {
        if (tid < nv) vU[tid] = vEst[tid] < INFINITY ? fmaxf(vEst[tid], vLb[tid]) : INFINITY;
        __syncthreads();
        if (tid < nv) {
            const float my = vU[tid];
            uint32_t rk = 0;
            for (uint32_t j = 0; j < nv; ++j) { const float o = vU[j]; rk += (o < my || (o == my && j < tid)) ? 1u : 0u; }
            if (rk == top_k - 1u) res[0] = my;
        }
        __syncthreads();
        const float r = res[0];
        __syncthreads();
        return r;
    }
    const uint32_t R0 = (uint32_t)RBQ_HX_REFINE_MULT * top_k > 16u ? (uint32_t)RBQ_HX_REFINE_MULT * top_k : 16u;
    const uint32_t R = R0 < nv ? R0 : nv;
    if (tid < nv) {
        const float my = vEst[tid];
        uint32_t rk = 0;
        for (uint32_t j = 0; j < nv; ++j) { const float o = vEst[j]; rk += (o < my || (o == my && j < tid)) ? 1u : 0u; }
        if (rk < R) hist[rk] = tid;
    }
    __syncthreads();
    {
        const uint32_t grp = tid >> 4, gl = tid & 15u;
        const uint32_t nunits = ex_w4(D, ex_bits);
        const size_t exb = ex_bytes_dev(D, ex_bits);
        for (uint32_t j = grp; j < R; j += kThreads / 16) {
            uint32_t v = hist[j];
            if (v >= nv) { if (gl == 0 && P.fallback_count) atomicAdd(P.fallback_count + 2, 1u); v = 0; }
            const uint32_t slot = (gb + (v >> 5)) * 32u + (v & 31u);
            const uint8_t* ex = P.ex_codes + (size_t)slot * exb;
            const float fa = P.f_add_ex[slot], fr = P.f_rescale_ex[slot];
            float sacc;
            if constexpr (V != kVarAvx512) sacc = ex_dot_var_rt<V>(ex, sq, gl, nunits, D / 16, ex_bits);
            else if (RBQ_HX_EX_ALL && nunits <= (uint32_t)kExRegUnits) {
                uint4 uu[kExRegUnits];
                ex_load_all(uu, ex, gl, nunits);
                sacc = ex_bits == 6 ? ex_dot_all<6>(uu, sq, gl, nunits) : ex_dot_all<2>(uu, sq, gl, nunits);
            } else sacc = ex_bits == 6 ? ex_dot_units<6>(ex, sq, gl, nunits) : ex_dot_units<2>(ex, sq, gl, nunits);
            if constexpr (V == kVarAvx512) sacc = group16_reduce(sacc);
            if (gl == 0) {
                float tt2 = qc.scale * vIp[v];
                const float t0 = tt2;
                tt2 = tt2 + sacc;
                const float t1 = tt2;
                tt2 = tt2 + qc.kbx;
                const float a = fa + g_add;
                const float m = fr * tt2;
                const float d = a + m;
                const bool ok = vEst[v] < INFINITY && hx_tame(fa) && hx_tame(fr) && hx_tame(t0) && hx_tame(sacc) && hx_tame(t1) && hx_tame(tt2) &&
                                hx_tame(a) && hx_tame(m) && hx_tame(d);
                vU[j] = ok ? fmaxf(d, vLb[v]) : INFINITY;
            }
        }
    }
    __syncthreads();
    if (tid < R) {
        const float my = vU[tid];
        uint32_t rk = 0;
        for (uint32_t j = 0; j < R; ++j) { const float o = vU[j]; rk += (o < my || (o == my && j < tid)) ? 1u : 0u; }
        if (rk == top_k - 1u) res[0] = my;
    }
    __syncthreads();
    const float r = res[0];
    __syncthreads();
    return r;
}

constexpr uint32_t kSelHead = 4;
constexpr uint32_t kSelTodoMax = 512;
constexpr uint32_t kSelKeptMax = 256;
constexpr uint32_t kSelZoneMax = 1024;

template <int RM, int V = kVarAvx512>
__global__ RBQ_SEL_BOUNDS void k_select_mfma(const SelectParams P, const SelectGeom G) {
    extern __shared__ __align__(16) unsigned char smraw[];
    const uint32_t nlist = P.nlist, nprobe = P.nprobe, cap2 = G.cap2, D = P.D;
    const int metric = P.metric;
    uint64_t* keys = reinterpret_cast<uint64_t*>(smraw);
    float* qrot = reinterpret_cast<float*>(smraw + (size_t)cap2 * 8);
    uint32_t* part = reinterpret_cast<uint32_t*>(qrot + D);
    __shared__ uint32_t hist[256];
    __shared__ uint32_t s_k, s_cnt, s_bad;
    __shared__ unsigned long long s_nvec;
#ifdef RBQ_SEL_STAMPS
    unsigned long long ts[8]; int tn = 0;
#define SSTAMP() ts[tn++] = __builtin_amdgcn_s_memtime()
#else
#define SSTAMP()
#endif
#if defined(RBQ_SEL_STAMPS) && RBQ_SEL_STAMPS == 4
    unsigned long long ls[8] = {0, 0, 0, 0, 0, 0, 0, 0};
#define LSTAMP(i) ls[i] = __builtin_amdgcn_s_memtime()
#else
#define LSTAMP(i)
#endif
    SSTAMP();
    const uint32_t q = blockIdx.x, tid = threadIdx.x;
    float* grow = P.scores + (size_t)q * nlist;
    float* lrow = reinterpret_cast<float*>(part + kThreads);
    uint32_t* pgeo = reinterpret_cast<uint32_t*>(lrow + (RM == 1 ? nlist : 0u));
    float* rows = reinterpret_cast<float*>(smraw + ((reinterpret_cast<unsigned char*>(pgeo + (G.stage ? 4u * nprobe : 0u)) - smraw + 15) & ~(size_t)15));
    constexpr int KPT = 16;
    uint32_t kreg[KPT];
    bool bad_load = false;
    uint64_t* cand = reinterpret_cast<uint64_t*>(pgeo);
    bool use_cand = false;
    uint32_t n_cand = 0;
    auto okey = [&](float s) -> uint32_t {
        int32_t k = total_key(s);
        if (metric == 1) k = ~k;
        return (uint32_t)k ^ 0x80000000u;
    };
    auto cost_of = [&](uint32_t k32) -> float {
        int32_t k = (int32_t)(k32 ^ 0x80000000u);
        if (metric == 1) k = ~k;
        const float s = key_to_float(k);
        return metric == 0 ? s : -s;
    };
    if (RM == 2) {
#pragma unroll
        for (int v = 0; v < KPT / 4; ++v) {
            const uint32_t i = v * 1024u + tid * 4u;
            float4 x = make_float4(0, 0, 0, 0);
            if (i + 3 < nlist) x = *reinterpret_cast<const float4*>(grow + i);
            else { if (i < nlist) x.x = grow[i]; if (i + 1 < nlist) x.y = grow[i + 1]; if (i + 2 < nlist) x.z = grow[i + 2]; }
            bad_load |= !finite_f(x.x) || !finite_f(x.y) || !finite_f(x.z) || !finite_f(x.w);
            kreg[4 * v] = okey(x.x); kreg[4 * v + 1] = okey(x.y); kreg[4 * v + 2] = okey(x.z); kreg[4 * v + 3] = okey(x.w);
        }
    } else if (RM == 1) {
        for (uint32_t i = tid; i < nlist; i += kThreads) lrow[i] = grow[i];
    }
    auto each_key = [&](auto&& body) {
        if (RM == 2) {
#pragma unroll
            for (int u = 0; u < KPT; ++u) {
                const uint32_t i = (uint32_t)(u >> 2) * 1024u + tid * 4u + (uint32_t)(u & 3);
                if (i < nlist) body(i, kreg[u]);
            }
        } else if (RM == 1) {
            for (uint32_t i = tid; i < nlist; i += kThreads) { const float v = lrow[i]; bad_load |= !finite_f(v); body(i, okey(v)); }
        } else if (use_cand) {
            for (uint32_t j = tid; j < n_cand; j += kThreads) { const uint64_t kc = cand[j]; body((uint32_t)kc, (uint32_t)(kc >> 32)); }
        } else {
            for (uint32_t i = tid; i < nlist; i += kThreads) { const float v = grow[i]; bad_load |= !finite_f(v); body(i, okey(v)); }
        }
    };

    {
        float qv[4];
        for (uint32_t i0 = tid; i0 < D; i0 += 4 * kThreads) {
#pragma unroll
            for (int u = 0; u < 4; ++u) qv[u] = i0 + (uint32_t)u * kThreads < D ? P.rot[(size_t)q * D + i0 + (uint32_t)u * kThreads] : 0.0f;
#pragma unroll
            for (int u = 0; u < 4; ++u) if (i0 + (uint32_t)u * kThreads < D) qrot[i0 + (uint32_t)u * kThreads] = qv[u];
        }
    }
    if (tid == 0) { s_k = nprobe - 1; s_cnt = 0; s_nvec = 0; s_bad = 0; }
    __syncthreads();

    SSTAMP();
    bool all = nprobe >= nlist;
    __shared__ uint32_t s_lo, s_hi, s_bin, s_cum, s_h, s_ng, s_w4[4], s_nc;
    auto kth_key = [&](auto&& each, uint32_t k) -> uint32_t {
        if (tid == 0) { s_lo = 0xffffffffu; s_hi = 0u; s_ng = 0u; }
        __syncthreads();
        {
            uint32_t kmn = 0xffffffffu, kmx = 0u;
            each([&](uint32_t, uint32_t key) {
                kmn = key < kmn ? key : kmn;
                kmx = key > kmx ? key : kmx;
            });
            const bool bad = bad_load;
            kmn = wave_min_u32(kmn);
            kmx = ~wave_min_u32(~kmx);
            if ((tid & 63u) == 0) { atomicMin(&s_lo, kmn); atomicMax(&s_hi, kmx); }
            if (bad) s_bad = 1;
        }
        __syncthreads();
        uint32_t lo = s_lo, hi = s_hi;
        while (true) {
            const uint32_t span = hi - lo;
            const uint32_t sh = span < 256u ? 0u : (32u - (uint32_t)__builtin_clz(span)) - 8u;
            hist[tid] = 0;
            __syncthreads();
            each([&](uint32_t, uint32_t key) {
                if (key - lo <= hi - lo) atomicAdd(&hist[(key - lo) >> sh], 1u);
            });
            __syncthreads();
            const uint32_t h = hist[tid];
            uint32_t total;
            const uint32_t excl = block_scan_excl256(h, s_w4, tid, total);
            if (excl <= k && k < excl + h) { s_bin = tid; s_cum = excl; s_h = h; }
            __syncthreads();
            k -= s_cum;
            lo += s_bin << sh;
            const uint32_t width = (sh ? (1u << sh) : 1u) - 1u;
            if (hi - lo > width) hi = lo + width;
            if (sh == 0) break;
            const uint32_t nc = s_h;
            if (nc <= (uint32_t)kThreads) {
                uint32_t* cnd = hist;
                each([&](uint32_t, uint32_t key) {
                    if (key - lo <= hi - lo) cnd[atomicAdd(&s_ng, 1u)] = key;
                });
                __syncthreads();
                if (tid < nc) {
                    const uint32_t my = cnd[tid];
                    uint32_t less = 0, eq = 0;
#pragma unroll 8
                    for (uint32_t j = 0; j < nc; ++j) {
                        const uint32_t kj = cnd[j];
                        less += kj < my ? 1u : 0u;
                        eq += kj == my ? 1u : 0u;
                    }
                    if (less <= k && k < less + eq) s_lo = my;
                }
                __syncthreads();
                lo = s_lo;
                break;
            }
        }
        __syncthreads();
        return lo;
    };
    const QueryConsts qc = P.consts[q];
    const float eps = ((6.0f * (float)D + 16.0f) * 5.9604645e-8f + 4.0f * 1.52587890625e-5f) * (qc.qnorm2 + P.cnorm2_max) * 1.001f;
    auto widen = [&](uint32_t key) -> uint32_t {
        int32_t k = (int32_t)(key ^ 0x80000000u);
        if (metric == 1) k = ~k;
        const float sc = key_to_float(k);
        const float lim = metric == 0 ? sc + 2.0f * eps : sc - 2.0f * eps;
        return finite_f(lim) ? okey(lim) : 0xffffffffu;
    };
    constexpr int KL = 8;
    if (RM == 0 && !all && G.cand_cap >= 4u * nprobe && 2u * nprobe <= (uint32_t)(kThreads * KL)) {
        uint32_t lk[KL];
#pragma unroll
        for (int u = 0; u < KL; ++u) lk[u] = 0xffffffffu;
        constexpr int KU = 8;
        for (uint32_t i0 = tid; i0 < nlist; i0 += kThreads * KU) {
            float vv[KU];
#pragma unroll
            for (int w = 0; w < KU; ++w) { const uint32_t i = i0 + (uint32_t)w * kThreads; vv[w] = i < nlist ? grow[i] : 0.0f; }
#pragma unroll
            for (int w = 0; w < KU; ++w) {
                if (i0 + (uint32_t)w * kThreads < nlist) {
                    const float v = vv[w];
                    bad_load |= !finite_f(v);
                    const uint32_t key = okey(v);
                    if (key < lk[KL - 1]) {
                        lk[KL - 1] = key;
#pragma unroll
                        for (int u = KL - 1; u > 0; --u) {
                            const uint32_t a = lk[u - 1], b = lk[u];
                            lk[u - 1] = a < b ? a : b;
                            lk[u] = a < b ? b : a;
                        }
                    }
                }
            }
        }
        const uint32_t B = kth_key([&](auto&& body) {
#pragma unroll
            for (int u = 0; u < KL; ++u) if (lk[u] != 0xffffffffu) body(0u, lk[u]);
        }, nprobe - 1);
        const uint32_t cutB = widen(B);
        if (tid == 0) s_nc = 0;
        __syncthreads();
        if (cutB != 0xffffffffu && s_bad == 0) {
            for (uint32_t i0 = tid; i0 < nlist; i0 += kThreads * KU) {
                float vv[KU];
#pragma unroll
                for (int w = 0; w < KU; ++w) { const uint32_t i = i0 + (uint32_t)w * kThreads; vv[w] = i < nlist ? grow[i] : 0.0f; }
#pragma unroll
                for (int w = 0; w < KU; ++w) {
                    const uint32_t i = i0 + (uint32_t)w * kThreads;
                    const uint32_t key = okey(vv[w]);
                    if (i < nlist && key <= cutB) {
                        const uint32_t pp = atomicAdd(&s_nc, 1u);
                        if (pp < G.cand_cap) cand[pp] = ((uint64_t)key << 32) | i;
                    }
                }
            }
            __syncthreads();
            n_cand = s_nc;
            use_cand = n_cand <= G.cand_cap && n_cand >= nprobe;
        }
        __syncthreads();
    }
    uint32_t tau_key = 0;
    if (!all) tau_key = kth_key(each_key, nprobe - 1);
    else {
        each_key([&](uint32_t, uint32_t) {});
        if (bad_load) s_bad = 1;
        __syncthreads();
    }
    SSTAMP();
    const uint32_t cut = all ? 0xffffffffu : widen(tau_key);
    __shared__ uint32_t s_cntle, s_minab;
    for (uint32_t i = tid; i < cap2; i += kThreads) keys[i] = ~0ull;
    __shared__ uint32_t s_z0, s_tub, s_flag, s_need, s_dead, s_maxh, s_nh, s_nk, s_head[kSelHead];
    __shared__ unsigned long long s_memvec;
    if (tid == 0) { s_cntle = 0; s_minab = 0xffffffffu;
                    s_z0 = 0; s_tub = (uint32_t)total_key(INFINITY); s_flag = 0; s_need = 0; s_dead = 0; s_maxh = (uint32_t)total_key(-INFINITY); s_memvec = 0; s_nh = 0; s_nk = 0; }
    if (tid < kSelHead) s_head[tid] = 0xffffffffu;
    __syncthreads();
    bool fallback = s_bad != 0 || P.force_fallback != 0;
    if (!fallback) {
        uint32_t cle = 0, mab = 0xffffffffu;
        each_key([&](uint32_t i, uint32_t key) {
            if (key <= cut) {
                const uint32_t p = atomicAdd(&s_cnt, 1u);
                if (p < cap2) keys[p] = ((uint64_t)key << 32) | i;
                if (all || key <= tau_key) ++cle;
                else mab = key < mab ? key : mab;
            }
        });
        cle = wave_sum_u32(cle);
        mab = wave_min_u32(mab);
        if ((tid & 63u) == 0) { if (cle) atomicAdd(&s_cntle, cle); if (mab != 0xffffffffu) atomicMin(&s_minab, mab); }
        __syncthreads();
        fallback = s_cnt > cap2 || s_cnt < nprobe;
    }
    __syncthreads();
    SSTAMP();
    const uint32_t l2 = tid & 1u, grp = tid >> 1;
    uint32_t m_scan = nprobe;
    uint32_t dbg_tub = 0x7fc00000u, dbg_z = 0;
    uint32_t dead_vec = 0;
    if (!fallback) {
        const uint32_t n = s_cnt;
        LSTAMP(0);
        __shared__ uint32_t s_wmin[4][kSelHead], s_todo[kSelTodoMax];
        const uint32_t nown = (n + kThreads - 1 - tid) / kThreads;
        unsigned long long m_certain = 0ull, m_dead = 0ull, m_apx = 0ull;
        BlockSummary ls_own = {0.0f, 0.0f, 0.0f, 0.0f, 0.0f, 0.0f, 0u, 0u};
        uint32_t gb_own = 0, n_own = 0;
        float cn_own = 0.0f;
        if (P.lazy && tid < n) {
            const uint32_t cid = (uint32_t)keys[tid];
            ls_own = P.lsum[cid]; gb_own = P.list_gb0[cid]; n_own = P.list_n[cid];
            if (metric == 1) cn_own = P.cnorm2[cid];
        }
        const uint32_t bound_key = (!all && s_cntle > nprobe) ? tau_key : s_minab;
        const float cost_bound = (all || bound_key == 0xffffffffu) ? INFINITY : cost_of(bound_key);
        {
            uint32_t cnt = 0;
            for (uint32_t u = 0; u < nown && tid < n; ++u) {
                const uint32_t k32 = (uint32_t)(keys[tid + u * kThreads] >> 32);
                if (all || k32 <= tau_key) m_apx |= 1ull << u;
                const bool cert = cost_of(k32) + 2.01f * eps < cost_bound;
                if (cert) { m_certain |= 1ull << u; ++cnt; }
            }
            cnt = wave_sum_u32(cnt);
            if ((tid & 63u) == 0 && cnt) atomicAdd(&s_z0, cnt);
        }
        {
            uint32_t prev = 0;
            const uint32_t wave = tid >> 6;
#pragma unroll
            for (uint32_t r = 0; r < kSelHead; ++r) {
                uint32_t best = 0xffffffffu;
                for (uint32_t u = 0; u < nown && tid < n; ++u) {
                    const uint32_t k32 = (uint32_t)(keys[tid + u * kThreads] >> 32);
                    if ((r == 0 || k32 > prev) && k32 < best) best = k32;
                }
                best = wave_min_u32(best);
                if ((tid & 63u) == 0) s_wmin[wave][r] = best;
                prev = best;
            }
        }
        __syncthreads();
        const uint32_t z0 = s_z0;
#ifdef RBQ_PREP_STAMPS
        const bool lazy_ok = false;
#else
        const bool lazy_ok = P.lazy != 0 && z0 > 0 && n - z0 <= kSelZoneMax && qc.amax <= 65535.0f && P.top_k > 0;
#endif
        uint32_t h = 0;
        if (lazy_ok) {
            uint32_t prev = 0, lvl = 0xffffffffu;
#pragma unroll
            for (uint32_t r = 0; r < kSelHead; ++r) {
                uint32_t best = 0xffffffffu;
#pragma unroll
                for (int w = 0; w < 4; ++w)
#pragma unroll
                    for (uint32_t j = 0; j < kSelHead; ++j) {
                        const uint32_t v = s_wmin[w][j];
                        if ((r == 0 || v > prev) && v < best) best = v;
                    }
                if (best != 0xffffffffu) lvl = best;
                prev = best;
            }
            for (uint32_t u = 0; u < nown && tid < n; ++u) {
                const uint32_t i = tid + u * kThreads;
                if (((m_certain >> u) & 1ull) && (uint32_t)(keys[i] >> 32) <= lvl) {
                    const uint32_t p = atomicAdd(&s_nh, 1u);
                    if (p < kSelHead) s_head[p] = i;
                }
            }
            __syncthreads();
            h = s_nh < kSelHead ? s_nh : kSelHead;
        }
        const uint32_t hp0 = lazy_ok ? s_head[0] : 0xffffffffu, hp1 = lazy_ok ? s_head[1] : 0xffffffffu,
                       hp2 = lazy_ok ? s_head[2] : 0xffffffffu, hp3 = lazy_ok ? s_head[3] : 0xffffffffu;
        auto is_head = [&](uint32_t i) { return i == hp0 || i == hp1 || i == hp2 || i == hp3; };
        bool lazy = false;
        LSTAMP(1);
        if (lazy_ok && h > 0) {
            __shared__ uint32_t s_hgb[kSelHead], s_hn[kSelHead];
            __shared__ float s_hcn[kSelHead];
            if (tid < kSelHead) { s_hgb[tid] = 0; s_hn[tid] = 0; s_hcn[tid] = 0.0f; }
            if (tid == 0) s_need = h;
            __syncthreads();
#pragma unroll
            for (uint32_t r = 0; r < kSelHead; ++r) {
                const uint32_t pos = r == 0 ? hp0 : r == 1 ? hp1 : r == 2 ? hp2 : hp3;
                if (r < h && (pos & (kThreads - 1)) == tid) {
                    uint32_t gb = gb_own, nv = n_own;
                    float cn = cn_own;
                    if (pos >= (uint32_t)kThreads) { const uint32_t cid = (uint32_t)keys[pos]; gb = P.list_gb0[cid]; nv = P.list_n[cid]; if (metric == 1) cn = P.cnorm2[cid]; }
                    s_hgb[r] = gb; s_hn[r] = nv; s_hcn[r] = cn;
                }
            }
            __syncthreads();
            LSTAMP(2);
            auto head_info = [&](uint32_t r, float& g_add, float& g_err, uint32_t& gb, uint32_t& nvec) {
                const uint64_t key = keys[s_head[r]];
                const float ci = cost_of((uint32_t)(key >> 32));
                g_add = ci + 1.01f * eps;
                if (metric == 0) g_err = sqrtf(fmaxf(g_add, 0.0f));
                else g_err = sqrtf(fmaxf(qc.qnorm2 + s_hcn[r] + 2.0f * ci + 4.0f * eps, 0.0f));
                gb = s_hgb[r]; nvec = s_hn[r];
            };
            const uint32_t nb0 = (s_hn[0] + 31u) >> 5, nb1 = (s_hn[1] + 31u) >> 5, nb2 = (s_hn[2] + 31u) >> 5, nb3 = (s_hn[3] + 31u) >> 5;
            static_assert(kSelHead == 4, "four head lists");
            const uint32_t tot = nb0 + nb1 + nb2 + nb3;
            const uint32_t ncand = tot < (uint32_t)kThreads ? tot : (uint32_t)kThreads;
            float myU = INFINITY;
            uint32_t myN = 0;
            if (tid < ncand) {
                uint32_t r = 0, b = tid;
                if (b >= nb0) { b -= nb0; r = 1; if (b >= nb1) { b -= nb1; r = 2; if (b >= nb2) { b -= nb2; r = 3; } } }
                float g_add, g_err; uint32_t gb, nvec;
                head_info(r, g_add, g_err, gb, nvec);
                const BlockSummary bs = P.bsum[gb + b];
                const BlockSummaryEx bx = P.bsumx[gb + b];
                myU = block_ub(bs, bx, g_add, g_err, qc, D, P.ex_bits, P.slack, V == kVarPortable) + 1e-4f * eps;
                myN = (b + 1 == ((nvec + 31u) >> 5)) ? nvec - b * 32u : 32u;
                if (P.head_ub) {
                    uint32_t* hu = P.head_ub + (size_t)q * kHeadUbRow + 10 + 3 * tid;
                    hu[0] = gb + b; hu[1] = __float_as_uint(myU); hu[2] = myN;
                }
            }
            float* candU = reinterpret_cast<float*>(part);
            candU[tid] = myU; hist[tid] = myN;
            if (tid < h) {
                float g_add, g_err; uint32_t gb, nvec;
                head_info(tid, g_add, g_err, gb, nvec);
                if (P.head_ub) {
                    uint32_t* hu = P.head_ub + (size_t)q * kHeadUbRow;
                    hu[2 + 2 * tid] = __float_as_uint(g_add); hu[3 + 2 * tid] = __float_as_uint(g_err);
                    if (tid == 0) { hu[0] = ncand; hu[1] = h; }
                }
                atomicMax(reinterpret_cast<int*>(&s_maxh), total_key(g_add));
            }
            __syncthreads();
            if (tid < ncand && myU < INFINITY) {
                uint32_t cum = 0;
#pragma unroll 8
                for (uint32_t j = 0; j < ncand; ++j) cum += candU[j] <= myU ? hist[j] : 0u;
                if (cum >= P.top_k) atomicMin(reinterpret_cast<int*>(&s_tub), total_key(myU));
            }
            __syncthreads();
            float T_ub = P.fault_dead_all ? -INFINITY : key_to_float((int32_t)s_tub);
            const float cost_maxh = key_to_float((int32_t)s_maxh);
            bool hx_done = false;
            if (P.filter) {
                T_ub = (G.hx_nv && P.head_exact) ? head_exact_bound<V>(P, G, qc, keys, s_head, s_hgb, s_hn, s_hcn, h, eps, reinterpret_cast<unsigned char*>(rows), qrot, part, hist, q, tid, cost_of) : INFINITY;
                hx_done = true;
                if (P.fault_dead_all) T_ub = -INFINITY;
            }
            lazy = T_ub < INFINITY;
            dbg_tub = __float_as_uint(T_ub);
            if (tid < h) s_todo[tid] = s_head[tid];
            LSTAMP(3);
            if (lazy) {
                auto classify = [&](float T) {
                    for (uint32_t u = 0; u < nown && tid < n; ++u) {
                        const uint32_t i = tid + u * kThreads;
                        if (is_head(i)) continue;
                        const uint64_t key = keys[i];
                        const uint32_t cid = (uint32_t)key;
                        const float ci = cost_of((uint32_t)(key >> 32));
                        const float clo = ci - 1.01f * eps, chi = ci + 1.01f * eps;
                        float ge_lo, ge_hi;
                        if (metric == 0) { ge_lo = sqrtf(fmaxf(clo, 0.0f)); ge_hi = sqrtf(fmaxf(chi, 0.0f)); }
                        else {
                            const float da = qc.qnorm2 + (u == 0 ? cn_own : P.cnorm2[cid]) + 2.0f * ci;
                            ge_lo = sqrtf(fmaxf(da - 4.0f * eps, 0.0f)); ge_hi = sqrtf(fmaxf(da + 4.0f * eps, 0.0f));
                        }
                        const BlockSummary ls = u == 0 ? ls_own : P.lsum[cid];
                        const bool dead = clo > cost_maxh && list_bound_reaches(ls, clo, chi, ge_lo, ge_hi, qc, T, V == kVarPortable);
                        if (dead) m_dead |= 1ull << u;
                        else {
                            if (!((m_certain >> u) & 1ull)) s_flag = 1u;
                            const uint32_t p = atomicAdd(&s_need, 1u);
                            if (p < kSelTodoMax) s_todo[p] = i;
                        }
                    }
                    __syncthreads();
                };
                classify(T_ub);
                const uint32_t need1 = s_need;
                __syncthreads();
                if (G.hx_nv && P.head_exact && !hx_done && need1 - h > kHxTrigger) {
                    const float T2 = head_exact_bound<V>(P, G, qc, keys, s_head, s_hgb, s_hn, s_hcn, h, eps, reinterpret_cast<unsigned char*>(rows), qrot, part, hist, q, tid, cost_of);
                    if (T2 < T_ub) {
                        m_dead = 0ull;
                        if (tid == 0) { s_need = h; s_flag = 0u; }
                        __syncthreads();
                        classify(T2);
                        dbg_tub = __float_as_uint(T2);
                    }
                }
                const bool zone_scored = s_flag != 0u || P.exact_members != 0;
                if (zone_scored) {
                    for (uint32_t u = 0; u < nown && tid < n; ++u) {
                        const uint32_t i = tid + u * kThreads;
                        if (!is_head(i) && ((m_dead >> u) & 1ull) && !((m_certain >> u) & 1ull)) {
                            const uint32_t p = atomicAdd(&s_need, 1u);
                            if (p < kSelTodoMax) s_todo[p] = i;
                        }
                    }
                    __syncthreads();
                }
                LSTAMP(4);
                lazy = s_need <= kSelTodoMax;
                dbg_z = (z0 & 0x3ffu) | ((n & 0x3ffu) << 10) | (((s_need - h) & 0xfffu) << 20);
                if (lazy) {
                    const uint32_t m = s_need;
                    if (m) {
                        auto todo_idx = [&](uint32_t j) { return s_todo[j]; };
                        if (G.stage_rows && m <= 2u * G.stage_rows) canon_score_staged(keys, qrot, P.cent, D, metric, grow, m, tid, rows, G.stage_rows, todo_idx);
                        else {
                            if (m <= 64u) canon_score_octets(keys, qrot, P.cent, D, metric, grow, m, tid, todo_idx);
                            else canon_score_pairs(keys, qrot, P.cent, D, metric, grow, m, tid, todo_idx);
                            __threadfence_block();
                            __syncthreads();
                        }
                    }
                    LSTAMP(5);
                    __shared__ uint32_t s_zone[512];
                    __shared__ unsigned long long s_kept[kSelKeptMax];
                    if (zone_scored) {
                        for (uint32_t w = tid; w < 512; w += kThreads) s_zone[w] = 0u;
                        __syncthreads();
                        for (uint32_t u = 0; u < nown && tid < n; ++u)
                            if (!((m_certain >> u) & 1ull)) { const uint32_t i = tid + u * kThreads; atomicOr(&s_zone[i >> 5], 1u << (i & 31u)); }
                        __syncthreads();
                    }
                    unsigned long long m_keep = 0ull;
                    uint32_t dv = 0;
                    unsigned long long mv = 0;
                    for (uint32_t u = 0; u < nown && tid < n; ++u) {
                        const uint32_t i = tid + u * kThreads;
                        const bool cert = (m_certain >> u) & 1ull, dead = (m_dead >> u) & 1ull;
                        bool member = cert;
                        if (!cert && zone_scored) {
                            const uint64_t my = keys[i];
                            uint32_t less = 0;
                            for (uint32_t j = 0; j < n; ++j) less += ((s_zone[j >> 5] >> (j & 31u)) & 1u) && keys[j] < my ? 1u : 0u;
                            member = less < nprobe - z0;
                        }
                        if (dead && P.audit_dead) {
                            uint32_t* ad = P.audit_dead + (size_t)q * (kAuditCap + 1);
                            const uint32_t pa = atomicAdd(ad, 1u);
                            if (pa < kAuditCap) ad[1 + pa] = (uint32_t)keys[i];
                        }
                        if (member && !dead) {
                            m_keep |= 1ull << u;
                            const uint32_t p = atomicAdd(&s_nk, 1u);
                            if (p < kSelKeptMax) s_kept[p] = keys[i];
                        }
                        if (P.exact_members ? member : (P.prof_total != nullptr && ((m_apx >> u) & 1ull))) {
                            const uint32_t nvec = P.list_n[(uint32_t)keys[i]];
                            mv += nvec;
                            if (dead && P.exact_members) dv += nvec;
                        }
                    }
                    if (dv) atomicAdd(&s_dead, dv);
                    if (mv) atomicAdd(&s_memvec, mv);
                    __syncthreads();
                    if (s_nk <= kSelKeptMax) {
                        m_scan = s_nk;
                        if (tid < m_scan) {
                            const unsigned long long my = s_kept[tid];
                            uint32_t rk = 0;
#pragma unroll 4
                            for (uint32_t j = 0; j < m_scan; ++j) rk += s_kept[j] < my ? 1u : 0u;
                            keys[rk] = my;
                        }
                        __syncthreads();
                    } else {
                        uint32_t base = 0;
                        for (uint32_t c0 = 0, u = 0; c0 < n; c0 += kThreads, ++u) {
                            const uint32_t i = c0 + tid;
                            const bool keep = i < n && ((m_keep >> u) & 1ull);
                            const uint64_t v = i < n ? keys[i] : ~0ull;
                            uint32_t total;
                            const uint32_t off = block_scan_excl256(keep ? 1u : 0u, s_w4, tid, total);
                            if (keep) keys[base + off] = v;
                            base += total;
                        }
                        __syncthreads();
                        m_scan = base;
                        for (uint32_t i = m_scan + tid; i < cap2; i += kThreads) keys[i] = ~0ull;
                        __syncthreads();
                        sort_keys(keys, m_scan, cap2, tid);
                    }
                    LSTAMP(6);
                    if (tid == 0) dead_vec = s_dead;
                }
            }
        }
        if (!lazy) {
            auto all_idx = [](uint32_t j) { return j; };
            canon_score_pairs(keys, qrot, P.cent, D, metric, grow, n, tid, all_idx);
            __syncthreads();
            SSTAMP();
            sort_keys(keys, n, cap2, tid);
        }
#ifdef RBQ_SEL_STAMPS
        else SSTAMP();
#endif
    } else {
        if (tid == 0 && P.fallback_count) atomicAdd(P.fallback_count, 1u);
        float* row = grow;
        for (uint32_t base = 0; base < nlist; base += kThreads / 2) {
            const uint32_t cid = base + grp;
            if (cid < nlist) {
                const float* c = P.cent + (size_t)cid * D;
                const float s = metric == 0 ? canon_pair2<0>(qrot, c, D, l2) : canon_pair2<1>(qrot, c, D, l2);
                if (l2 == 0) row[cid] = s;
            }
        }
        __threadfence_block();
        __syncthreads();
        __shared__ unsigned long long s_prefix64, s_mask64;
        if (tid == 0) { s_prefix64 = all ? ~0ull : 0ull; s_mask64 = 0; s_k = nprobe - 1; s_cnt = 0; }
        __syncthreads();
        if (!all) {
            for (int pass = 7; pass >= 0; --pass) {
                const int shift = pass * 8;
                hist[tid] = 0;
                __syncthreads();
                const unsigned long long prefix = s_prefix64, mask = s_mask64;
                for (uint32_t i = tid; i < nlist; i += kThreads) {
                    const uint64_t key = make_key(row[i], i, metric);
                    if ((key & mask) == prefix) atomicAdd(&hist[(uint32_t)(key >> shift) & 255u], 1u);
                }
                __syncthreads();
                if (tid == 0) {
                    uint32_t k = s_k, cum = 0, bb = 0;
                    for (; bb < 256; ++bb) {
                        const uint32_t h = hist[bb];
                        if (k < cum + h) break;
                        cum += h;
                    }
                    s_k = k - cum;
                    s_prefix64 = prefix | ((unsigned long long)bb << shift);
                    s_mask64 = mask | (0xffull << shift);
                }
                __syncthreads();
            }
        }
        const uint64_t kstar = s_prefix64;
        for (uint32_t i = tid; i < cap2; i += kThreads) keys[i] = ~0ull;
        __syncthreads();
        for (uint32_t i = tid; i < nlist; i += kThreads) {
            const uint64_t key = make_key(row[i], i, metric);
            if (key <= kstar) {
                const uint32_t p = atomicAdd(&s_cnt, 1u);
                if (p < cap2) keys[p] = key;
            }
        }
        __syncthreads();
        for (uint32_t k = 2; k <= cap2; k <<= 1)
            for (uint32_t j = k >> 1; j > 0; j >>= 1) {
                for (uint32_t i = tid; i < cap2; i += kThreads) {
                    const uint32_t ixj = i ^ j;
                    if (ixj > i) {
                        const uint64_t a = keys[i], b2 = keys[ixj];
                        const bool up = (i & k) == 0;
                        if ((a > b2) == up) { keys[i] = b2; keys[ixj] = a; }
                    }
                }
                __syncthreads();
            }
    }

    SSTAMP();
    const uint32_t np = m_scan;
    float* dist_ip = reinterpret_cast<float*>(keys + nprobe);
    if (metric == 1 && !fallback) {
        __threadfence_block();
        __syncthreads();
        const volatile float* vrow = grow;
        for (uint32_t r = tid; r < np; r += kThreads) {
            dist_ip[r] = vrow[(uint32_t)(keys[r] & 0xffffffffu)];
        }
        __syncthreads();
    } else if (metric == 1) {
        for (uint32_t i0 = 0; i0 < np; i0 += kThreads / 2) {
            const uint32_t r = i0 + grp;
            float d = 0.0f;
            if (r < np) {
                const uint32_t cid = (uint32_t)(keys[r] & 0xffffffffu);
                d = canon_pair2<0>(qrot, P.cent + (size_t)cid * D, D, l2);
            }
            __syncthreads();
            if (r < np && l2 == 0) dist_ip[r] = d;
        }
        __syncthreads();
    }
    auto probe_consts = [&](uint32_t r) -> ProbeInfo {
        const uint64_t key = keys[r];
        int32_t k = (int32_t)((uint32_t)(key >> 32) ^ 0x80000000u);
        if (metric == 1) k = ~k;
        const float s = key_to_float(k);
        float dist, dot;
        if (metric == 0) { dist = s; dot = 0.0f; }
        else { dot = s; dist = dist_ip[r]; }
        ProbeInfo pi;
        pi.g_add = metric == 0 ? dist : -dot;
        pi.g_err = sqrtf(dist);
        pi.dotqc = dot;
        pi.cid = (uint32_t)(key & 0xffffffffu);
        return pi;
    };
    uint32_t* pstart = reinterpret_cast<uint32_t*>(dist_ip + nprobe);
    const uint32_t per = (np + kThreads - 1) / kThreads;
    const uint32_t r0 = tid * per < np ? tid * per : np, r1 = (r0 + per < np) ? r0 + per : np;
    uint32_t local = 0;
    unsigned long long local_vec = 0;
    for (uint32_t r = r0; r < r1; ++r) {
        const ProbeInfo pi = probe_consts(r);
        P.probe[(size_t)q * nprobe + r] = pi;
        const uint32_t n = P.list_n[pi.cid];
        if (G.stage) {
            pgeo[r] = __float_as_uint(pi.g_add);
            pgeo[nprobe + r] = __float_as_uint(pi.g_err);
            pgeo[2 * nprobe + r] = P.list_gb0[pi.cid];
            pgeo[3 * nprobe + r] = n;
        }
        local += (n + 31u) >> 5;
        local_vec += n;
    }
    if (local_vec) atomicAdd(&s_nvec, local_vec);
    uint32_t run;
    uint32_t acc0 = block_scan_excl256(local, s_w4, tid, run);
    for (uint32_t r = r0; r < r1; ++r) {
        pstart[r] = acc0;
        acc0 += ((G.stage ? pgeo[3 * nprobe + r] : P.list_n[(uint32_t)(keys[r] & 0xffffffffu)]) + 31u) >> 5;
    }
    if (tid == 0) {
        P.nstream[q] = run;
        const unsigned long long nv = np == nprobe ? s_nvec : s_memvec;
        P.nvec[q] = nv;
        if (P.prof_total) atomicAdd(P.prof_total + prof_stripe(q), nv);
        if (P.dead_skipped) {
            P.dead_skipped[q] = dead_vec; P.dead_skipped[P.nq + q] = np;
            P.dead_skipped[2 * (size_t)P.nq + q] = dbg_tub; P.dead_skipped[3 * (size_t)P.nq + q] = dbg_z;
        }
    }
    __syncthreads();
    StreamItem* out = P.wl + (size_t)q * P.wl_stride;
    for (uint32_t base = 0; base < run; base += 4 * kThreads) {
        uint32_t rr[4], gbb[4], nvv[4];
        BlockSummary bs[4];
#pragma unroll
        for (int u = 0; u < 4; ++u) {
            const uint32_t i = base + u * kThreads + tid;
            rr[u] = 0; gbb[u] = 0; nvv[u] = 0;
// ... 130 lines not shown
```

### rabitq-rs_amd/index.py

```python
import ctypes as C
import os

import numpy as np

from . import _abi

_HERE = os.path.dirname(os.path.abspath(__file__))
_LIB = None
LIB_PATH = os.environ.get("RBQ_LIB_PATH") or os.path.join(_HERE, "csrc", "librbq.so")


def _hip_runtime_of_torch_first():
    import sys
    if "torch" not in sys.modules:
        try:
            import torch
        except ImportError:
            pass


def lib():
    global _LIB
    if _LIB is None:
        if not os.path.exists(LIB_PATH):
            raise RuntimeError(
                f"{LIB_PATH} missing: the HIP extension must be built first "
                "(python -c 'import __graft_entry__ as g; g.build()'); there is no CPU fallback")
        _hip_runtime_of_torch_first()
        L = C.CDLL(LIB_PATH)
        vp = C.c_void_p
        L.rbq_index_create.restype = C.c_int
        L.rbq_index_create.argtypes = [vp, vp, C.c_int, vp, C.POINTER(vp)]
        L.rbq_index_load_rbq1.restype = C.c_int
        L.rbq_index_load_rbq1.argtypes = [vp, C.c_size_t, C.c_int, vp, C.POINTER(vp)]
        L.rbq_index_destroy.argtypes = [vp]
        for n in ("rbq_index_len", "rbq_index_cluster_count"):
            getattr(L, n).restype = C.c_uint64
            getattr(L, n).argtypes = [vp]
        for n in ("rbq_index_dim", "rbq_index_padded_dim"):
            getattr(L, n).restype = C.c_uint32
            getattr(L, n).argtypes = [vp]
        L.rbq_search_batch.restype = C.c_int
        L.rbq_search_batch.argtypes = [vp, vp, C.c_uint64, C.c_uint32, C.c_uint32, C.c_uint32, vp, C.c_uint64,
                                       vp, vp, vp, vp]
        L.rbq_search_batch_device.restype = C.c_int
        L.rbq_search_batch_device.argtypes = [vp, vp, C.c_uint64, C.c_uint32, C.c_uint32, C.c_uint32, vp,
                                              C.c_uint64, vp, vp, vp, vp, vp]
        L.rbq_posting_scan_batch.restype = C.c_int
        L.rbq_posting_scan_batch.argtypes = [vp, vp, C.c_uint64, C.c_uint32, C.c_uint32, vp, vp, C.c_uint32, vp, vp, vp]
        L.rbq_profile_begin.argtypes = [vp]
        L.rbq_profile_end.argtypes = [vp]
        L.rbq_profile_stage_ms.restype = C.c_double
        L.rbq_profile_stage_ms.argtypes = [vp, C.c_char_p, C.POINTER(C.c_uint64)]
        L.rbq_profile_scan_bytes.restype = C.c_uint64
        L.rbq_profile_scan_bytes.argtypes = [vp]
        L.rbq_debug_rank_fallbacks.restype = C.c_uint64
        L.rbq_debug_rank_fallbacks.argtypes = [vp]
        L.rbq_debug_stage_resources.restype = C.c_int
        L.rbq_debug_stage_resources.argtypes = [vp, C.c_uint64, C.c_uint32, C.c_uint32, vp]
        for n_ in ("rbq_debug_head_exact_evaluations", "rbq_debug_head_exact_guard_trips"):
            getattr(L, n_).restype = C.c_uint64
            getattr(L, n_).argtypes = [vp]
        L.rbq_debug_tie_log_stats.restype = None
        L.rbq_debug_tie_log_stats.argtypes = [vp, vp]
        L.rbq_debug_bounce_copies.restype = C.c_uint64
        L.rbq_debug_bounce_copies.argtypes = []
        L.rbq_index_build_device.restype = C.c_int
        L.rbq_index_build_device.argtypes = [vp, vp, vp, vp, C.c_uint64, C.c_float, C.c_int, vp]
        L.rbq_index_build_device_ex.restype = C.c_int
        L.rbq_index_build_device_ex.argtypes = [vp, vp, vp, vp, C.c_uint64, C.c_int, C.c_float, C.c_int, vp]
        L.rbq_debug_best_rescale.restype = C.c_int
        L.rbq_debug_best_rescale.argtypes = [vp, C.c_uint64, C.c_uint32, C.c_uint32, C.c_int, vp]
        L.rbq_debug_copy_index.restype = C.c_int
        L.rbq_debug_copy_index.argtypes = [vp, C.c_char_p, vp, C.c_uint64]
        L.rbq_profile_set_sampling.restype = None
        L.rbq_profile_set_sampling.argtypes = [vp, C.c_uint32]
        L.rbq_profile_select_stages.restype = None
        L.rbq_profile_select_stages.argtypes = [vp, C.c_uint32]
        L.rbq_debug_copy_workspace.restype = C.c_int
        L.rbq_debug_copy_workspace.argtypes = [vp, vp, C.c_char_p, vp, C.c_uint64]
        L.rbq_debug_heap_restarts.restype = C.c_uint64
        L.rbq_debug_heap_restarts.argtypes = [vp]
        L.rbq_debug_set_option.restype = C.c_int
        L.rbq_debug_set_option.argtypes = [vp, C.c_char_p, C.c_int]
        L.rbq_strerror.restype = C.c_char_p
        L.rbq_strerror.argtypes = [C.c_int]
        L.rbq_last_error_detail.restype = C.c_int
        L.rbq_last_error_detail.argtypes = [C.c_char_p, C.c_size_t]
        L.rbq_abi_version.restype = C.c_uint32
        L.rbq_index_device_count.restype = C.c_uint32
        L.rbq_index_device_count.argtypes = [vp]
        L.rbq_build_stream_begin.restype = C.c_int
        L.rbq_build_stream_begin.argtypes = [vp, vp, vp, C.c_float, C.c_int, C.POINTER(vp)]
        L.rbq_build_stream_begin_ex.restype = C.c_int
        L.rbq_build_stream_begin_ex.argtypes = [vp, vp, vp, C.c_int, C.c_float, C.c_int, C.POINTER(vp)]
        L.rbq_build_stream_push.restype = C.c_int
        L.rbq_build_stream_push.argtypes = [vp, vp, vp, C.c_uint64, C.c_uint64]
        L.rbq_build_stream_finish.restype = C.c_int
        L.rbq_build_stream_finish.argtypes = [vp, C.c_int, vp, C.POINTER(vp)]
        L.rbq_build_stream_abort.restype = None
        L.rbq_build_stream_abort.argtypes = [vp]
        L.rbq_release_stream.restype = C.c_int
        L.rbq_release_stream.argtypes = [vp, vp]
        L.rbq_host_alloc.restype = vp
        L.rbq_host_alloc.argtypes = [C.c_size_t]
        L.rbq_host_free.restype = None
        L.rbq_host_free.argtypes = [vp]
        L.rbq_index_set_rerank_vectors.restype = C.c_int
        L.rbq_index_set_rerank_vectors.argtypes = [vp, vp, C.c_uint64]
        L.rbq_profile_stage_samples.restype = C.c_uint64
        L.rbq_profile_stage_samples.argtypes = [vp, C.c_char_p, vp, C.c_uint64]
        L.rbq_profile_counters.restype = C.c_int
        L.rbq_profile_counters.argtypes = [vp, vp, C.c_uint32]
        L.rbq_index_set_numeric_variant.restype = C.c_int
        L.rbq_index_set_numeric_variant.argtypes = [vp, C.c_int]
        L.rbq_index_numeric_variant.restype = C.c_int
        L.rbq_index_numeric_variant.argtypes = [vp]
        L.rbq_kmeans_device.restype = C.c_int
        L.rbq_kmeans_device.argtypes = [vp, C.c_uint64, C.c_uint32, C.c_uint64, C.c_uint64, C.c_uint64, C.c_uint64, C.c_int,
                                        C.c_uint64, C.c_uint64, C.c_int, vp, vp, C.POINTER(C.c_double), vp]
        L.rbq_index_create_with_recon.restype = C.c_int
        L.rbq_index_create_with_recon.argtypes = [vp, vp, vp, vp, C.c_int, vp, C.POINTER(vp)]
        L.rbq_index_save_rbq1_stream.restype = C.c_int
        L.rbq_index_save_rbq1_stream.argtypes = [vp, WRITE_FN, vp]
        L.rbq_index_save_rbq1.restype = C.c_int
        L.rbq_index_save_rbq1.argtypes = [vp, C.POINTER(C.POINTER(C.c_uint8)), C.POINTER(C.c_uint64)]
        L.rbq_persist_free_bytes.restype = None
        L.rbq_persist_free_bytes.argtypes = [C.POINTER(C.c_uint8)]
        L.rbq_debug_crc32_device.restype = C.c_int
        L.rbq_debug_crc32_device.argtypes = [vp, C.c_uint64, C.c_int, C.POINTER(C.c_uint32)]
        L.rbq_index_fetch_embeddings.restype = C.c_int
        L.rbq_index_fetch_embeddings.argtypes = [vp, vp, C.c_uint64, vp, vp]
        L.rbq_index_fetch_embeddings_device.restype = C.c_int
        L.rbq_index_fetch_embeddings_device.argtypes = [vp, vp, C.c_uint64, vp, vp, vp]
        L.rbq_mstg_closure_assign.restype = C.c_int
        L.rbq_mstg_closure_assign.argtypes = [vp, C.c_uint64, C.c_uint32, vp, C.c_uint64, C.c_float, C.c_uint32, C.c_uint64, C.c_int,
                                              vp, vp]
        L.rbq_mstg_build_device.restype = C.c_int
        L.rbq_mstg_build_device.argtypes = [vp, vp, vp, C.c_uint64, C.c_float, C.c_uint32, C.c_int, C.c_float, C.c_uint64, C.c_int,
                                            C.POINTER(vp)]
        L.rbq_mstg_debug_closure_fallbacks.restype = C.c_uint64
        L.rbq_mstg_debug_closure_fallbacks.argtypes = []
        L.rbq_mstg_debug_closure_shortlist.restype = C.c_int
        L.rbq_mstg_debug_closure_shortlist.argtypes = [vp, C.c_uint64, C.c_uint32, vp, C.c_uint64, C.c_uint32, C.c_uint64, C.c_int,
                                                       vp, vp]
        L.rbq_mstg_search_batch.restype = C.c_int
        L.rbq_mstg_search_batch.argtypes = [vp, vp, C.c_uint64, C.c_uint32, C.c_uint32, C.c_uint32, C.c_float, vp, vp, vp, vp, vp]
        L.rbq_mstg_search_batch_device.restype = C.c_int
        L.rbq_mstg_search_batch_device.argtypes = [vp, vp, C.c_uint64, C.c_uint32, C.c_uint32, C.c_uint32, C.c_float, vp, vp, vp, vp, vp,
                                                   vp]
        L.rbq_mstg_search_refined_batch.restype = C.c_int
        L.rbq_mstg_search_refined_batch.argtypes = [vp, vp, C.c_uint64, C.c_uint32, C.c_uint32, C.c_uint32, C.c_float, C.c_uint32, vp, vp, vp,
                                                    vp, vp]
        L.rbq_mstg_search_refined_batch_device.restype = C.c_int
        L.rbq_mstg_search_refined_batch_device.argtypes = [vp, vp, C.c_uint64, C.c_uint32, C.c_uint32, C.c_uint32, C.c_float, C.c_uint32, vp,
                                                           vp, vp, vp, vp, vp]
        L.rbq_mstg_debug_search_fallbacks.restype = C.c_uint64
        L.rbq_mstg_debug_search_fallbacks.argtypes = []
        L.rbq_mstg_cluster_device.restype = C.c_int
        L.rbq_mstg_cluster_device.argtypes = [vp, C.c_uint64, C.c_uint32, C.c_uint64, C.c_uint64, C.c_float, C.c_uint64, C.c_uint64,
                                              C.c_int, C.POINTER(vp)]
        L.rbq_mstg_save_stream.restype = C.c_int
        L.rbq_mstg_save_stream.argtypes = [vp, vp, WRITE_FN, vp]
        L.rbq_mstg_save.restype = C.c_int
        L.rbq_mstg_save.argtypes = [vp, vp, C.POINTER(C.POINTER(C.c_uint8)), C.POINTER(C.c_uint64)]
        L.rbq_mstg_load.restype = C.c_int
        L.rbq_mstg_load.argtypes = [vp, C.c_uint64, C.c_int, vp, C.POINTER(vp)]
        L.rbq_mstg_load_stream.restype = C.c_int
        L.rbq_mstg_load_stream.argtypes = [READ_FN, vp, C.c_uint64, C.c_int, vp, C.POINTER(vp)]
        L.rbq_mstg_memory_usage.restype = C.c_uint64
        L.rbq_mstg_memory_usage.argtypes = [vp]
        from .builder import bind_hclustered
        bind_hclustered(L)
        _LIB = L
    return _LIB


WRITE_FN = C.CFUNCTYPE(C.c_int, C.c_void_p, C.c_void_p, C.c_uint64)
READ_FN = C.CFUNCTYPE(C.c_int, C.c_void_p, C.c_uint64, C.c_void_p, C.c_uint64)


def _detail():
    buf = C.create_string_buffer(512)
    lib().rbq_last_error_detail(buf, 512)
    return buf.value.decode("utf-8", "replace")


def _check(rc):
    if rc != _abi.RBQ_OK:
        from . import RabitqError
        raise RabitqError(rc, _detail())


def _rescale(mode, t_const):
    m = _abi.RESCALE_MODES.get(mode, -1) if isinstance(mode, str) else int(mode)
    return m, float(t_const) if t_const is not None else 0.0


def _addr(ptr):
    return C.cast(ptr, C.c_void_p)


class IvfRabitqIndex:

    def __init__(self, handle):
        self._h = handle

    @staticmethod
    def _devices(device, devices):
        if devices is not None:
            devices = list(devices)
            return len(devices), (C.c_int * len(devices))(*devices)
        return 1, ((C.c_int * 1)(device) if device is not None else None)

    @classmethod
    def from_built(cls, built, device=None, devices=None):
        from . import builder
# ... 138 lines not shown
        _check(lib().rbq_debug_crc32_device(C.c_void_p(d_ptr), int(n), int(device), C.byref(out)))
        return out.value

    def fetch_embeddings(self, ids):
        q = np.ascontiguousarray(np.asarray(ids, dtype=np.uint64).reshape(-1))
        n = int(q.size)
        out = np.empty((n, self.dim), np.float32)
        found = np.empty(n, np.uint8)
        _check(lib().rbq_index_fetch_embeddings(self._h, q.ctypes.data, n, out.ctypes.data, found.ctypes.data))
        return out, found.astype(bool)

    def fetch_embedding(self, vector_id):
        out, found = self.fetch_embeddings([vector_id])
        return out[0] if found[0] else None

    def fetch_embeddings_device(self, d_ids, n, d_out, d_found, stream=None):
        _check(lib().rbq_index_fetch_embeddings_device(self._h, C.c_void_p(d_ids), int(n), C.c_void_p(d_out), C.c_void_p(d_found),
                                                       C.c_void_p(stream) if stream else None))

    def __len__(self):
        return lib().rbq_index_len(self._h)

    def is_empty(self):
        return len(self) == 0

    def cluster_count(self):
        return lib().rbq_index_cluster_count(self._h)

    @property
    def dim(self):
        return lib().rbq_index_dim(self._h)

    @property
    def padded_dim(self):
        return lib().rbq_index_padded_dim(self._h)

    def batch_search_raw(self, queries, params, filter_words=None, filter_nbits=0, want_diag=False):
        q = np.ascontiguousarray(queries, dtype=np.float32)
        if q.ndim == 1:
            q = q[None, :]
        nq, qd = q.shape
        k = params.top_k
        ids = np.empty((nq, k), np.uint64)
        scores = np.empty((nq, k), np.float32)
        counts = np.zeros(nq, np.uint32)
        diag = np.zeros((nq, 3), np.uint64) if want_diag else None
        fw = np.ascontiguousarray(filter_words, dtype=np.uint32) if filter_words is not None else None
        rc = lib().rbq_search_batch(self._h, q.ctypes.data, nq, qd, k, params.nprobe,
                                    fw.ctypes.data if fw is not None else None, filter_nbits,
                                    ids.ctypes.data, scores.ctypes.data, counts.ctypes.data,
                                    diag.ctypes.data if diag is not None else None)
        _check(rc)
        return ids, scores, counts, diag

    def _results(self, ids, scores, counts, q):
        from . import SearchResult
        return [SearchResult(int(ids[q, i]), float(scores[q, i])) for i in range(int(counts[q]))]

    def search(self, query, params):
        ids, scores, counts, _ = self.batch_search_raw(np.asarray(query, np.float32)[None, :], params)
        return self._results(ids, scores, counts, 0)

    def search_filtered(self, query, params, allowed_ids):
        allowed = np.asarray(sorted(set(int(i) for i in allowed_ids)), dtype=np.uint64)
        nbits = int(allowed.max()) + 1 if allowed.size else 0
        words = np.zeros((nbits + 31) // 32 or 1, np.uint32)
        if allowed.size:
            np.bitwise_or.at(words, (allowed >> np.uint64(5)).astype(np.int64),
                             (np.uint32(1) << (allowed & np.uint64(31)).astype(np.uint32)))
        ids, scores, counts, _ = self.batch_search_raw(np.asarray(query, np.float32)[None, :], params,
                                                       words, nbits)
        return self._results(ids, scores, counts, 0)

    def batch_search(self, queries, params):
        ids, scores, counts, _ = self.batch_search_raw(queries, params)
        return [self._results(ids, scores, counts, q) for q in range(ids.shape[0])]

    def batch_query(self, queries, top_k, nprobe):
        from . import SearchParams
        ids, scores, counts, _ = self.batch_search_raw(queries, SearchParams(top_k, nprobe))
        out = []
        for q in range(ids.shape[0]):
            c = int(counts[q])
            out.append(np.stack([ids[q, :c].astype(np.float32), scores[q, :c]], axis=1))
        return out

    def posting_scan(self, queries, top_k, list_ids, list_counts):
        q = np.ascontiguousarray(queries, dtype=np.float32)
        li = np.ascontiguousarray(list_ids, dtype=np.uint32)
        lc = np.ascontiguousarray(list_counts, dtype=np.uint32)
        nq, qd = q.shape
        ids = np.empty((nq, top_k), np.uint64)
        scores = np.empty((nq, top_k), np.float32)
        counts = np.zeros(nq, np.uint32)
        _check(lib().rbq_posting_scan_batch(self._h, q.ctypes.data, nq, qd, top_k, li.ctypes.data, lc.ctypes.data,
                                            li.shape[1], ids.ctypes.data, scores.ctypes.data, counts.ctypes.data))
        return ids, scores, counts

    def search_batch_device(self, d_queries, nq, query_dim, top_k, nprobe, d_ids, d_scores, d_counts,
                            stream=None, d_filter=None, filter_nbits=0, d_diag=None):
        _check(lib().rbq_search_batch_device(self._h, d_queries, nq, query_dim, top_k, nprobe, d_filter,
                                             filter_nbits, d_ids, d_scores, d_counts, d_diag, stream))

    def profile_begin(self, stages=("prep", "rank", "select", "scan"), every=1):
        mask = sum(1 << ("prep", "rank", "select", "scan").index(s) for s in stages)
        lib().rbq_profile_select_stages(self._h, mask)
        lib().rbq_profile_set_sampling(self._h, every)
        lib().rbq_profile_begin(self._h)

    def profile_end(self):
        lib().rbq_profile_end(self._h)

    def profile_stage(self, name):
        n = C.c_uint64()
        ms = lib().rbq_profile_stage_ms(self._h, name.encode(), C.byref(n))
        return ms, n.value

    def profile_stage_samples(self, name):
        n = lib().rbq_profile_stage_samples(self._h, name.encode(), None, 0)
        out = np.zeros(max(int(n), 1), np.float32)
        lib().rbq_profile_stage_samples(self._h, name.encode(), out.ctypes.data, int(n))
        return out[:int(n)]

    def set_option(self, name, value):
        _check(lib().rbq_debug_set_option(self._h, name.encode(), int(value)))

    def set_numeric_variant(self, variant):
        if isinstance(variant, str):
            if variant not in _abi.NUMERIC_VARIANTS:
                from . import RabitqError
                raise RabitqError(_abi.RBQ_INVALID_CONFIG, "unknown numeric variant %r (one of %s)" % (variant, ", ".join(_abi.NUMERIC_VARIANTS)))
            variant = _abi.NUMERIC_VARIANTS[variant]
        _check(lib().rbq_index_set_numeric_variant(self._h, int(variant)))

    @property
    def numeric_variant(self):
        v = lib().rbq_index_numeric_variant(self._h)
        return {i: n for n, i in _abi.NUMERIC_VARIANTS.items()}[v]

    def stage_resources(self, nq, top_k, nprobe):
        out = np.zeros((4, 6), np.uint32)
        _check(lib().rbq_debug_stage_resources(self._h, nq, top_k, nprobe, out.ctypes.data))
        return {s: {"workgroups": int(o[0]), "threads": int(o[1]), "vgprs": int(o[2]), "lds_bytes": int(o[3]), "scratch_bytes": int(o[4])}
                for s, o in zip(("prep", "rank", "select", "scan"), out)}

    def head_exact_stats(self):
        return int(lib().rbq_debug_head_exact_evaluations(self._h)), int(lib().rbq_debug_head_exact_guard_trips(self._h))

    def tie_log_stats(self):
        out = np.zeros(4, np.uint64)
        lib().rbq_debug_tie_log_stats(self._h, out.ctypes.data)
        return dict(zip(("replays", "entries", "heap_ops", "overflows"), (int(v) for v in out)))

    def rank_fallbacks(self):
        return lib().rbq_debug_rank_fallbacks(self._h)

    def debug_copy_workspace(self, stream, name, out):
        _check(lib().rbq_debug_copy_workspace(self._h, C.c_void_p(stream), name.encode(), out.ctypes.data, out.nbytes))
        return out

    def heap_restarts(self):
        return lib().rbq_debug_heap_restarts(self._h)

    def profile_scan_bytes(self):
        return lib().rbq_profile_scan_bytes(self._h)

    def device_count(self):
        return lib().rbq_index_device_count(self._h)

    def profile_counters(self):
        out = (C.c_uint64 * 8)()
        _check(lib().rbq_profile_counters(self._h, out, 8))
        names = ("vectors_probed", "code_blocks", "meta_blocks", "stream_entries", "ex_evals", "queries")
        return {k: int(out[i]) for i, k in enumerate(names)}

    def release_stream(self, stream):
        _check(lib().rbq_release_stream(self._h, C.c_void_p(stream)))

    def set_rerank_vectors(self, vectors=None, device_ptr=None, n=0):
        if device_ptr is not None:
            _check(lib().rbq_index_set_rerank_vectors(self._h, C.c_void_p(device_ptr), int(n)))
        elif vectors is None:
            _check(lib().rbq_index_set_rerank_vectors(self._h, None, 0))
        else:
            v = np.ascontiguousarray(vectors, dtype=np.float32)
            _check(lib().rbq_index_set_rerank_vectors(self._h, v.ctypes.data, v.shape[0]))

    def close(self):
        if self._h:
            lib().rbq_index_destroy(self._h)
            self._h = None

    def __del__(self):
        try:
            self.close()
        except Exception:
            pass


class StreamBuilder:

    def __init__(self, hdr_ptr, centroids, list_sizes, t_const=None, device=0, rescale="const"):
        cent = np.ascontiguousarray(centroids, dtype=np.float32)
        ls = np.ascontiguousarray(list_sizes, dtype=np.uint32)
        mode, t = _rescale(rescale, t_const)
        self._b = C.c_void_p()
        _check(lib().rbq_build_stream_begin_ex(_addr(hdr_ptr), cent.ctypes.data, ls.ctypes.data, mode, t, int(device),
                                               C.byref(self._b)))

    def push(self, vectors, assign, first_id, count=None):
        if isinstance(vectors, np.ndarray):
            v = np.ascontiguousarray(vectors, dtype=np.float32)
            a = np.ascontiguousarray(assign, dtype=np.uint32)
            _check(lib().rbq_build_stream_push(self._b, v.ctypes.data, a.ctypes.data, int(first_id), v.shape[0]))
        else:
            _check(lib().rbq_build_stream_push(self._b, C.c_void_p(vectors), C.c_void_p(assign), int(first_id), int(count)))

    def finish(self, devices=None):
        h = C.c_void_p()
        if devices is None:
            _check(lib().rbq_build_stream_finish(self._b, 1, None, C.byref(h)))
        else:
            devices = list(devices)
            _check(lib().rbq_build_stream_finish(self._b, len(devices), (C.c_int * len(devices))(*devices), C.byref(h)))
        self._b = None
        return IvfRabitqIndex(h)

    def abort(self):
        if self._b:
            lib().rbq_build_stream_abort(self._b)
            self._b = None

    def __del__(self):
        try:
            self.abort()
        except Exception:
            pass
```

Before: 7.722 million.

## Add select-front path pruning probe candidates with index-wide list bound before kth selection

```diff
diff --git a/include/rbq.h b/include/rbq.h
--- a/include/rbq.h
+++ b/include/rbq.h
@@ -133,6 +133,7 @@
 void rbq_profile_set_sampling(rbq_index* idx, uint32_t every);
 uint64_t rbq_debug_rank_fallbacks(const rbq_index* idx);
 void rbq_debug_tie_log_stats(const rbq_index* idx, uint64_t* out4);
+void rbq_debug_select_front_stats(const rbq_index* idx, uint64_t* out4);
 int rbq_debug_stage_resources(rbq_index* idx, uint64_t nq, uint32_t top_k, uint32_t nprobe, uint32_t* out);
 uint64_t rbq_debug_bounce_copies(void);
 uint64_t rbq_debug_head_exact_evaluations(const rbq_index* idx);
diff --git a/rabitq-rs_amd/csrc/device/api.hpp b/rabitq-rs_amd/csrc/device/api.hpp
--- a/rabitq-rs_amd/csrc/device/api.hpp
+++ b/rabitq-rs_amd/csrc/device/api.hpp
@@ -299,6 +299,8 @@
     bool ub_tap = false;
     bool lazy_audit = false;
     bool lazy_select = true;
+    bool select_front = true;
+    uint32_t select_front_cap = 0;
     uint32_t tie_log_cap = 0;
     bool tie_log = true;
     int latency_path = 1;
@@ -334,6 +336,7 @@
     Arr mr_slot_map, mr_blk_list;
     bool mr_ready = false;
     float cnorm2_max = 0.0f;
+    BlockSummary gsum = {0.0f, 0.0f, 0.0f, 0.0f, 0.0f, 0.0f, 0u, 0u};
     uint64_t n_raw = 0;
     bool raw_borrowed = false;
     bool rerank = false;
diff --git a/rabitq-rs_amd/csrc/device/api_index.hip b/rabitq-rs_amd/csrc/device/api_index.hip
--- a/rabitq-rs_amd/csrc/device/api_index.hip
+++ b/rabitq-rs_amd/csrc/device/api_index.hip
@@ -88,6 +88,21 @@
     return ix;
 }
 
+static BlockSummary index_summary(const BlockSummary* ls, uint32_t nlist) {
+    BlockSummary g = {INFINITY, -INFINITY, INFINITY, -INFINITY, INFINITY, -INFINITY, nlist ? 1u : 0u, 0u};
+    for (uint32_t c = 0; c < nlist; ++c) {
+        const BlockSummary& s = ls[c];
+        const bool fin = std::isfinite(s.fadd_min) && std::isfinite(s.fadd_max) && std::isfinite(s.fres_min) && std::isfinite(s.fres_max) &&
+                         std::isfinite(s.ferr_min) && std::isfinite(s.ferr_max);
+        if (!s.usable || !fin) g.usable = 0u;
+        g.fadd_min = std::min(g.fadd_min, s.fadd_min); g.fadd_max = std::max(g.fadd_max, s.fadd_max);
+        g.fres_min = std::min(g.fres_min, s.fres_min); g.fres_max = std::max(g.fres_max, s.fres_max);
+        g.ferr_min = std::min(g.ferr_min, s.ferr_min); g.ferr_max = std::max(g.ferr_max, s.ferr_max);
+    }
+    if (!g.usable) g.fadd_min = g.fadd_max = g.fres_min = g.fres_max = g.ferr_min = g.ferr_max = 0.0f;
+    return g;
+}
+
 int finish_replica(Replica* ix, const std::vector<uint32_t>& ln) {
     const uint32_t nlist = (uint32_t)ix->n_lists, D = ix->D;
     ix->h_list_n = ln;
@@ -115,8 +130,13 @@
                                   (const float*)ix->fres_ex.p, (const float*)ix->centroids.p, (const BlockSummary*)ix->bsum.p,
                                   (const uint32_t*)ix->list_gb0.p, (const uint32_t*)ix->list_n.p, nlist, D, ix->Dc, ix->ex_bits,
                                   (BlockSummaryEx*)ix->bsumx.p, (BlockSummary*)ix->lsum.p, 0));
-    if ((rc = alloc_arr(ix->fallbacks, 32))) return rc;
-    HIP_TRY(hipMemset(ix->fallbacks.p, 0, 32));
+    {
+        std::vector<BlockSummary> ls(nlist);
+        HIP_TRY(hipMemcpy(ls.data(), ix->lsum.p, (size_t)nlist * sizeof(BlockSummary), hipMemcpyDeviceToHost));
+        ix->gsum = index_summary(ls.data(), nlist);
+    }
+    if ((rc = alloc_arr(ix->fallbacks, kCounterWords * 4))) return rc;
+    HIP_TRY(hipMemset(ix->fallbacks.p, 0, kCounterWords * 4));
     if ((rc = alloc_arr(ix->prof, (size_t)kProfStripes * kProfSlots * 8))) return rc;
     HIP_TRY(hipMemset(ix->prof.p, 0, (size_t)kProfStripes * kProfSlots * 8));
     const char* e = std::getenv("RBQ_EXACT_RANK");
@@ -134,6 +154,8 @@
     else if (is("exact_rank")) exact_rank = v != 0;
     else if (is("exact_heap")) exact_heap = v != 0;
     else if (is("lazy_select")) lazy_select = v != 0;
+    else if (is("select_front")) select_front = v != 0;
+    else if (is("select_front_cap")) select_front_cap = v > 0 ? (uint32_t)v : 0u;
     else if (is("rank_tile")) rank_tile = v;
     else if (is("latency_path")) latency_path = v;
     else if (is("tie_log")) tie_log = v != 0;
@@ -222,7 +244,7 @@
     static_cast<Geometry&>(*ix) = *src;
     ix->device = dev;
     ix->n_vectors = src->n_vectors; ix->n_lists = src->n_lists; ix->n_blocks = src->n_blocks;
-    ix->cnorm2_max = src->cnorm2_max; ix->h_list_n = src->h_list_n; ix->nblk_desc_prefix = src->nblk_desc_prefix;
+    ix->cnorm2_max = src->cnorm2_max; ix->gsum = src->gsum; ix->h_list_n = src->h_list_n; ix->nblk_desc_prefix = src->nblk_desc_prefix;
     ix->opt = src->opt;
     for (size_t i = 0; i < sizeof(ix->arrays) / sizeof(ix->arrays[0]); ++i) {
         const Arr* s = src->arrays[i];
@@ -233,7 +255,7 @@
         if (e != hipSuccess) { free_replica(ix); return fail(RBQ_DEVICE, std::string("replicating the index: ") + hipGetErrorString(e)); }
         d->bytes = s->bytes;
     }
-    hipError_t e = hipMemset(ix->fallbacks.p, 0, 32);
+    hipError_t e = hipMemset(ix->fallbacks.p, 0, kCounterWords * 4);
     if (e == hipSuccess) e = hipMemset(ix->prof.p, 0, (size_t)kProfStripes * kProfSlots * 8);
     if (e != hipSuccess) { free_replica(ix); return fail(RBQ_DEVICE, hipGetErrorString(e)); }
     *out = ix;
@@ -677,6 +699,7 @@
 }
 uint64_t rbq_debug_rank_fallbacks(const rbq_index* h) { return read_counter(h, 0); }
 void rbq_debug_tie_log_stats(const rbq_index* h, uint64_t* out4) { if (out4) for (int i = 0; i < 4; ++i) out4[i] = read_counter(h, 4 + i); }
+void rbq_debug_select_front_stats(const rbq_index* h, uint64_t* out4) { if (out4) for (int i = 0; i < 4; ++i) out4[i] = read_counter(h, (int)kFrontCounters + i); }
 uint64_t rbq_debug_head_exact_guard_trips(const rbq_index* h) { return read_counter(h, 2); }
 uint64_t rbq_debug_head_exact_evaluations(const rbq_index* h) { return read_counter(h, 3); }
 
diff --git a/rabitq-rs_amd/csrc/device/api_search.hip b/rabitq-rs_amd/csrc/device/api_search.hip
--- a/rabitq-rs_amd/csrc/device/api_search.hip
+++ b/rabitq-rs_amd/csrc/device/api_search.hip
@@ -218,6 +218,7 @@
     sp.f_add_ex = (const float*)ix->fadd_ex.p; sp.f_rescale_ex = (const float*)ix->fres_ex.p; sp.Dc = Dc;
     sp.head_exact = ix->opt.head_exact ? 1 : 0;
     sp.n_blocks = (uint32_t)ix->n_blocks;
+    sp.gsum = ix->gsum; sp.select_front = ix->opt.select_front ? 1 : 0; sp.front_cap = ix->opt.select_front_cap;
     if (ix->opt.exact_rank || big_nprobe) {
         uint64_t* kw = nullptr;
         if (big_nprobe) {
diff --git a/rabitq-rs_amd/csrc/device/launch.hpp b/rabitq-rs_amd/csrc/device/launch.hpp
--- a/rabitq-rs_amd/csrc/device/launch.hpp
+++ b/rabitq-rs_amd/csrc/device/launch.hpp
@@ -103,7 +103,12 @@
     uint32_t* head_ub;
     uint32_t numeric_variant;
     int fault_dead_all;
-};
+    BlockSummary gsum;
+    int select_front;
+    uint32_t front_cap;
+};
+constexpr uint32_t kFrontCounters = 8;
+constexpr uint32_t kCounterWords = 12;
 uint32_t select_exact_np2(uint32_t nprobe);
 hipError_t launch_select_exact(const SelectParams& p, int device, hipStream_t s, uint64_t* key_window);
 hipError_t launch_select_mfma(const SelectParams& p, int device, hipStream_t s);
diff --git a/rabitq-rs_amd/csrc/device/rank_mfma.hpp b/rabitq-rs_amd/csrc/device/rank_mfma.hpp
--- a/rabitq-rs_amd/csrc/device/rank_mfma.hpp
+++ b/rabitq-rs_amd/csrc/device/rank_mfma.hpp
@@ -793,7 +793,7 @@
         const float s = key_to_float(k);
         return metric == 0 ? s : -s;
     };
-    if (RM == 2) {
+    auto load_keys = [&]() {
 #pragma unroll
         for (int v = 0; v < KPT / 4; ++v) {
             const uint32_t i = v * 1024u + tid * 4u;
@@ -803,7 +803,9 @@
             bad_load |= !finite_f(x.x) || !finite_f(x.y) || !finite_f(x.z) || !finite_f(x.w);
             kreg[4 * v] = okey(x.x); kreg[4 * v + 1] = okey(x.y); kreg[4 * v + 2] = okey(x.z); kreg[4 * v + 3] = okey(x.w);
         }
-    } else if (RM == 1) {
+    };
+    if (RM == 2) load_keys();
+    else if (RM == 1) {
         for (uint32_t i = tid; i < nlist; i += kThreads) lrow[i] = grow[i];
     }
     auto each_key = [&](auto&& body) {
@@ -964,42 +966,243 @@
         }
         __syncthreads();
     }
-    uint32_t tau_key = 0;
-    if (!all) tau_key = kth_key(each_key, nprobe - 1);
-    else {
-        each_key([&](uint32_t, uint32_t) {});
-        if (bad_load) s_bad = 1;
-        __syncthreads();
-    }
-    SSTAMP();
-    const uint32_t cut = all ? 0xffffffffu : widen(tau_key);
     __shared__ uint32_t s_cntle, s_minab;
-    for (uint32_t i = tid; i < cap2; i += kThreads) keys[i] = ~0ull;
     __shared__ uint32_t s_z0, s_tub, s_flag, s_need, s_dead, s_maxh, s_nh, s_nk, s_head[kSelHead];
     __shared__ unsigned long long s_memvec;
-    if (tid == 0) { s_cntle = 0; s_minab = 0xffffffffu;
-                    s_z0 = 0; s_tub = (uint32_t)total_key(INFINITY); s_flag = 0; s_need = 0; s_dead = 0; s_maxh = (uint32_t)total_key(-INFINITY); s_memvec = 0; s_nh = 0; s_nk = 0; }
-    if (tid < kSelHead) s_head[tid] = 0xffffffffu;
-    __syncthreads();
-    bool fallback = s_bad != 0 || P.force_fallback != 0;
-    if (!fallback) {
-        uint32_t cle = 0, mab = 0xffffffffu;
+    __shared__ uint32_t s_wmin[4][kSelHead], s_hgb[kSelHead], s_hn[kSelHead];
+    __shared__ unsigned long long s_kept[kSelKeptMax];
+    __shared__ float s_hcn[kSelHead];
+    BlockSummary ls_own = {0.0f, 0.0f, 0.0f, 0.0f, 0.0f, 0.0f, 0u, 0u};
+    uint32_t gb_own = 0, n_own = 0;
+    float cn_own = 0.0f;
+    auto head_level = [&]() -> uint32_t {
+        uint32_t prev = 0, lvl = 0xffffffffu;
+#pragma unroll
+        for (uint32_t r = 0; r < kSelHead; ++r) {
+            uint32_t best = 0xffffffffu;
+#pragma unroll
+            for (int w = 0; w < 4; ++w)
+#pragma unroll
+                for (uint32_t j = 0; j < kSelHead; ++j) {
+                    const uint32_t v = s_wmin[w][j];
+                    if ((r == 0 || v > prev) && v < best) best = v;
+                }
+            if (best != 0xffffffffu) lvl = best;
+            prev = best;
+        }
+        return lvl;
+    };
+    auto head_bound = [&](uint32_t h, uint32_t hp0, uint32_t hp1, uint32_t hp2, uint32_t hp3) {
+        if (tid < kSelHead) { s_hgb[tid] = 0; s_hn[tid] = 0; s_hcn[tid] = 0.0f; }
+        if (tid == 0) s_need = h;
+        __syncthreads();
+#pragma unroll
+        for (uint32_t r = 0; r < kSelHead; ++r) {
+            const uint32_t pos = r == 0 ? hp0 : r == 1 ? hp1 : r == 2 ? hp2 : hp3;
+            if (r < h && (pos & (kThreads - 1)) == tid) {
+                uint32_t gb = gb_own, nv = n_own;
+                float cn = cn_own;
+                if (pos >= (uint32_t)kThreads) { const uint32_t cid = (uint32_t)keys[pos]; gb = P.list_gb0[cid]; nv = P.list_n[cid]; if (metric == 1) cn = P.cnorm2[cid]; }
+                s_hgb[r] = gb; s_hn[r] = nv; s_hcn[r] = cn;
+            }
+        }
+        __syncthreads();
+        LSTAMP(2);
+        auto head_info = [&](uint32_t r, float& g_add, float& g_err, uint32_t& gb, uint32_t& nvec) {
+            const uint64_t key = keys[s_head[r]];
+            const float ci = cost_of((uint32_t)(key >> 32));
+            g_add = ci + 1.01f * eps;
+            if (metric == 0) g_err = sqrtf(fmaxf(g_add, 0.0f));
+            else g_err = sqrtf(fmaxf(qc.qnorm2 + s_hcn[r] + 2.0f * ci + 4.0f * eps, 0.0f));
+            gb = s_hgb[r]; nvec = s_hn[r];
+        };
+        const uint32_t nb0 = (s_hn[0] + 31u) >> 5, nb1 = (s_hn[1] + 31u) >> 5, nb2 = (s_hn[2] + 31u) >> 5, nb3 = (s_hn[3] + 31u) >> 5;
+        static_assert(kSelHead == 4, "four head lists");
+        const uint32_t tot = nb0 + nb1 + nb2 + nb3;
+        const uint32_t ncand = tot < (uint32_t)kThreads ? tot : (uint32_t)kThreads;
+        float myU = INFINITY;
+        uint32_t myN = 0;
+        if (tid < ncand) {
+            uint32_t r = 0, b = tid;
+            if (b >= nb0) { b -= nb0; r = 1; if (b >= nb1) { b -= nb1; r = 2; if (b >= nb2) { b -= nb2; r = 3; } } }
+            float g_add, g_err; uint32_t gb, nvec;
+            head_info(r, g_add, g_err, gb, nvec);
+            const BlockSummary bs = P.bsum[gb + b];
+            const BlockSummaryEx bx = P.bsumx[gb + b];
+            myU = block_ub(bs, bx, g_add, g_err, qc, D, P.ex_bits, P.slack, V == kVarPortable) + 1e-4f * eps;
+            myN = (b + 1 == ((nvec + 31u) >> 5)) ? nvec - b * 32u : 32u;
+            if (P.head_ub) {
+                uint32_t* hu = P.head_ub + (size_t)q * kHeadUbRow + 10 + 3 * tid;
+                hu[0] = gb + b; hu[1] = __float_as_uint(myU); hu[2] = myN;
+            }
+        }
+        float* candU = reinterpret_cast<float*>(part);
+        candU[tid] = myU; hist[tid] = myN;
+        if (tid < h) {
+            float g_add, g_err; uint32_t gb, nvec;
+            head_info(tid, g_add, g_err, gb, nvec);
+            if (P.head_ub) {
+                uint32_t* hu = P.head_ub + (size_t)q * kHeadUbRow;
+                hu[2 + 2 * tid] = __float_as_uint(g_add); hu[3 + 2 * tid] = __float_as_uint(g_err);
+                if (tid == 0) { hu[0] = ncand; hu[1] = h; }
+            }
+            atomicMax(reinterpret_cast<int*>(&s_maxh), total_key(g_add));
+        }
+        __syncthreads();
+        if (tid < ncand && myU < INFINITY) {
+            uint32_t cum = 0;
+#pragma unroll 8
+            for (uint32_t j = 0; j < ncand; ++j) cum += candU[j] <= myU ? hist[j] : 0u;
+            if (cum >= P.top_k) atomicMin(reinterpret_cast<int*>(&s_tub), total_key(myU));
+        }
+        __syncthreads();
+    };
+    bool front = false;
+#ifndef RBQ_PREP_STAMPS
+    if (RM == 2 && P.select_front != 0 && P.lazy != 0 && metric == 0 && !all && P.filter == nullptr && P.exact_members == 0 &&
+        P.prof_total == nullptr && P.audit_dead == nullptr && P.head_ub == nullptr && P.fault_dead_all == 0 && P.force_fallback == 0 &&
+        P.gsum.usable != 0 && P.top_k > 0 && qc.amax <= 65535.0f && finite_f(eps)) {
+        uint32_t wcap = cap2 < kSelTodoMax ? cap2 : kSelTodoMax;
+        if (P.front_cap && P.front_cap < wcap) wcap = P.front_cap;
+        for (uint32_t i = tid; i < cap2; i += kThreads) keys[i] = ~0ull;
+        if (tid == 0) { s_z0 = 0; s_tub = (uint32_t)total_key(INFINITY); s_flag = 0; s_need = 0; s_dead = 0; s_maxh = (uint32_t)total_key(-INFINITY);
+                        s_memvec = 0; s_nh = 0; s_nk = 0; s_hi = 0u; s_ng = 0u; }
+        if (tid < kSelHead) s_head[tid] = 0xffffffffu;
+        if (bad_load) s_bad = 1;
+        {
+            uint32_t prev = 0;
+            const uint32_t wave = tid >> 6;
+#pragma unroll
+            for (uint32_t r = 0; r < kSelHead; ++r) {
+                uint32_t best = 0xffffffffu;
+                each_key([&](uint32_t, uint32_t key) { if ((r == 0 || key > prev) && key < best) best = key; });
+                best = wave_min_u32(best);
+                if ((tid & 63u) == 0) s_wmin[wave][r] = best;
+                prev = best;
+            }
+        }
+        __syncthreads();
+        const uint32_t lvl = head_level();
         each_key([&](uint32_t i, uint32_t key) {
-            if (key <= cut) {
+            if (key <= lvl) {
                 const uint32_t p = atomicAdd(&s_cnt, 1u);
-                if (p < cap2) keys[p] = ((uint64_t)key << 32) | i;
-                if (all || key <= tau_key) ++cle;
-                else mab = key < mab ? key : mab;
+                if (p < wcap) keys[p] = ((uint64_t)key << 32) | i;
             }
         });
-        cle = wave_sum_u32(cle);
-        mab = wave_min_u32(mab);
-        if ((tid & 63u) == 0) { if (cle) atomicAdd(&s_cntle, cle); if (mab != 0xffffffffu) atomicMin(&s_minab, mab); }
-        __syncthreads();
-        fallback = s_cnt > cap2 || s_cnt < nprobe;
-    }
-    __syncthreads();
-    SSTAMP();
+        __syncthreads();
+        const uint32_t nh = s_cnt;
+        uint32_t why = s_bad != 0 ? 3u : nh > wcap ? 2u : 0u;
+        float T_ub = INFINITY, cost_maxh = 0.0f;
+        if (why == 0) {
+            const uint32_t h = nh < kSelHead ? nh : kSelHead;
+            if (tid < h) s_head[tid] = tid;
+            if (tid == 0) s_nh = h;
+            if (tid < nh) { const uint32_t cid = (uint32_t)keys[tid]; gb_own = P.list_gb0[cid]; n_own = P.list_n[cid]; }
+            head_bound(h, 0u, 1u, 2u, 3u);
+            load_keys();
+            T_ub = key_to_float((int32_t)s_tub);
+            cost_maxh = key_to_float((int32_t)s_maxh);
+            if (!(T_ub < INFINITY)) why = 3u;
+        }
+        if (why == 0) {
+            each_key([&](uint32_t i, uint32_t key) {
+                if (key > lvl) {
+                    const float ci = cost_of(key);
+                    const float clo = ci - 1.01f * eps, chi = ci + 1.01f * eps;
+                    const float ge_lo = sqrtf(fmaxf(clo, 0.0f)), ge_hi = sqrtf(fmaxf(chi, 0.0f));
+                    if (!(clo > cost_maxh && list_bound_reaches(P.gsum, clo, chi, ge_lo, ge_hi, qc, T_ub, V == kVarPortable))) {
+                        const uint32_t p = atomicAdd(&s_cnt, 1u);
+                        if (p < wcap) keys[p] = ((uint64_t)key << 32) | i;
+                    }
+                }
+            });
+            __syncthreads();
+            if (s_cnt > wcap) why = 2u;
+        }
+        if (why == 0) {
+            const uint32_t ng = s_cnt;
+            uint32_t mx = 0;
+            for (uint32_t e = tid; e < ng; e += kThreads) {
+                const uint64_t key = keys[e];
+                const uint32_t k32 = (uint32_t)(key >> 32);
+                bool alive = e < nh;
+                if (!alive) {
+                    const float ci = cost_of(k32);
+                    const float clo = ci - 1.01f * eps, chi = ci + 1.01f * eps;
+                    const float ge_lo = sqrtf(fmaxf(clo, 0.0f)), ge_hi = sqrtf(fmaxf(chi, 0.0f));
+                    const BlockSummary ls = P.lsum[(uint32_t)key];
+                    alive = !(clo > cost_maxh && list_bound_reaches(ls, clo, chi, ge_lo, ge_hi, qc, T_ub, V == kVarPortable));
+                    if (alive) {
+                        const uint32_t p = atomicAdd(&s_nk, 1u);
+                        if (p < kSelKeptMax) s_kept[p] = key;
+                    }
+                }
+                if (alive) mx = k32 > mx ? k32 : mx;
+            }
+            mx = ~wave_min_u32(~mx);
+            if ((tid & 63u) == 0) atomicMax(&s_hi, mx);
+            __syncthreads();
+            const uint32_t na = s_nk;
+            if (na > kSelKeptMax || nh + na > wcap) why = 2u;
+            else {
+                for (uint32_t e = nh + tid; e < ng; e += kThreads) keys[e] = e - nh < na ? s_kept[e - nh] : ~0ull;
+                const float lim = cost_of(s_hi) + 2.01f * eps;
+                const uint32_t cut_m = finite_f(lim) ? okey(lim) : 0xffffffffu;
+                uint32_t cnt = 0;
+                each_key([&](uint32_t, uint32_t key) { cnt += key <= cut_m ? 1u : 0u; });
+                cnt = wave_sum_u32(cnt);
+                if ((tid & 63u) == 0) atomicAdd(&s_ng, cnt);
+                __syncthreads();
+                if (cut_m == 0xffffffffu || s_ng > nprobe) why = 1u;
+                else if (tid == 0) { s_cnt = nh + na; s_nk = 0; }
+            }
+        }
+        front = why == 0;
+        __syncthreads();
+        if (tid == 0) {
+            if (!front) s_cnt = 0;
+            if (P.fallback_count) atomicAdd(P.fallback_count + kFrontCounters + why, 1u);
+        }
+    }
+#endif
+    uint32_t tau_key = 0;
+    bool fallback = false;
+    if (!front) {
+        if (!all) tau_key = kth_key(each_key, nprobe - 1);
+        else {
+            each_key([&](uint32_t, uint32_t) {});
+            if (bad_load) s_bad = 1;
+            __syncthreads();
+        }
+        SSTAMP();
+        const uint32_t cut = all ? 0xffffffffu : widen(tau_key);
+        for (uint32_t i = tid; i < cap2; i += kThreads) keys[i] = ~0ull;
+        if (tid == 0) { s_cntle = 0; s_minab = 0xffffffffu;
+                        s_z0 = 0; s_tub = (uint32_t)total_key(INFINITY); s_flag = 0; s_need = 0; s_dead = 0; s_maxh = (uint32_t)total_key(-INFINITY); s_memvec = 0; s_nh = 0; s_nk = 0; }
+        if (tid < kSelHead) s_head[tid] = 0xffffffffu;
+        __syncthreads();
+        fallback = s_bad != 0 || P.force_fallback != 0;
+        if (!fallback) {
+            uint32_t cle = 0, mab = 0xffffffffu;
+            each_key([&](uint32_t i, uint32_t key) {
+                if (key <= cut) {
+                    const uint32_t p = atomicAdd(&s_cnt, 1u);
+                    if (p < cap2) keys[p] = ((uint64_t)key << 32) | i;
+                    if (all || key <= tau_key) ++cle;
+                    else mab = key < mab ? key : mab;
+                }
+            });
+            cle = wave_sum_u32(cle);
+            mab = wave_min_u32(mab);
+            if ((tid & 63u) == 0) { if (cle) atomicAdd(&s_cntle, cle); if (mab != 0xffffffffu) atomicMin(&s_minab, mab); }
+            __syncthreads();
+            fallback = s_cnt > cap2 || s_cnt < nprobe;
+        }
+        __syncthreads();
+        SSTAMP();
+    } else {
+        SSTAMP(); SSTAMP();
+    }
     const uint32_t l2 = tid & 1u, grp = tid >> 1;
     uint32_t m_scan = nprobe;
     uint32_t dbg_tub = 0x7fc00000u, dbg_z = 0;
@@ -1007,19 +1210,16 @@
     if (!fallback) {
         const uint32_t n = s_cnt;
         LSTAMP(0);
-        __shared__ uint32_t s_wmin[4][kSelHead], s_todo[kSelTodoMax];
+        __shared__ uint32_t s_todo[kSelTodoMax];
         const uint32_t nown = (n + kThreads - 1 - tid) / kThreads;
         unsigned long long m_certain = 0ull, m_dead = 0ull, m_apx = 0ull;
-        BlockSummary ls_own = {0.0f, 0.0f, 0.0f, 0.0f, 0.0f, 0.0f, 0u, 0u};
-        uint32_t gb_own = 0, n_own = 0;
-        float cn_own = 0.0f;
         if (P.lazy && tid < n) {
             const uint32_t cid = (uint32_t)keys[tid];
             ls_own = P.lsum[cid]; gb_own = P.list_gb0[cid]; n_own = P.list_n[cid];
             if (metric == 1) cn_own = P.cnorm2[cid];
         }
         const uint32_t bound_key = (!all && s_cntle > nprobe) ? tau_key : s_minab;
-        const float cost_bound = (all || bound_key == 0xffffffffu) ? INFINITY : cost_of(bound_key);
+        const float cost_bound = (front || all || bound_key == 0xffffffffu) ? INFINITY : cost_of(bound_key);
         {
             uint32_t cnt = 0;
             for (uint32_t u = 0; u < nown && tid < n; ++u) {
@@ -1031,7 +1231,7 @@
             cnt = wave_sum_u32(cnt);
             if ((tid & 63u) == 0 && cnt) atomicAdd(&s_z0, cnt);
         }
-        {
+        if (!front) {
             uint32_t prev = 0;
             const uint32_t wave = tid >> 6;
 #pragma unroll
@@ -1054,21 +1254,8 @@
         const bool lazy_ok = P.lazy != 0 && z0 > 0 && n - z0 <= kSelZoneMax && qc.amax <= 65535.0f && P.top_k > 0;
 #endif
         uint32_t h = 0;
-        if (lazy_ok) {
-            uint32_t prev = 0, lvl = 0xffffffffu;
-#pragma unroll
-            for (uint32_t r = 0; r < kSelHead; ++r) {
-                uint32_t best = 0xffffffffu;
-#pragma unroll
-                for (int w = 0; w < 4; ++w)
-#pragma unroll
-                    for (uint32_t j = 0; j < kSelHead; ++j) {
-                        const uint32_t v = s_wmin[w][j];
-                        if ((r == 0 || v > prev) && v < best) best = v;
-                    }
-                if (best != 0xffffffffu) lvl = best;
-                prev = best;
-            }
+        if (lazy_ok && !front) {
+            const uint32_t lvl = head_level();
             for (uint32_t u = 0; u < nown && tid < n; ++u) {
                 const uint32_t i = tid + u * kThreads;
                 if (((m_certain >> u) & 1ull) && (uint32_t)(keys[i] >> 32) <= lvl) {
@@ -1077,79 +1264,15 @@
                 }
             }
             __syncthreads();
-            h = s_nh < kSelHead ? s_nh : kSelHead;
-        }
+        }
+        if (lazy_ok) h = s_nh < kSelHead ? s_nh : kSelHead;
         const uint32_t hp0 = lazy_ok ? s_head[0] : 0xffffffffu, hp1 = lazy_ok ? s_head[1] : 0xffffffffu,
                        hp2 = lazy_ok ? s_head[2] : 0xffffffffu, hp3 = lazy_ok ? s_head[3] : 0xffffffffu;
         auto is_head = [&](uint32_t i) { return i == hp0 || i == hp1 || i == hp2 || i == hp3; };
         bool lazy = false;
         LSTAMP(1);
         if (lazy_ok && h > 0) {
-            __shared__ uint32_t s_hgb[kSelHead], s_hn[kSelHead];
-            __shared__ float s_hcn[kSelHead];
-            if (tid < kSelHead) { s_hgb[tid] = 0; s_hn[tid] = 0; s_hcn[tid] = 0.0f; }
-            if (tid == 0) s_need = h;
-            __syncthreads();
-#pragma unroll
-            for (uint32_t r = 0; r < kSelHead; ++r) {
-                const uint32_t pos = r == 0 ? hp0 : r == 1 ? hp1 : r == 2 ? hp2 : hp3;
-                if (r < h && (pos & (kThreads - 1)) == tid) {
-                    uint32_t gb = gb_own, nv = n_own;
-                    float cn = cn_own;
-                    if (pos >= (uint32_t)kThreads) { const uint32_t cid = (uint32_t)keys[pos]; gb = P.list_gb0[cid]; nv = P.list_n[cid]; if (metric == 1) cn = P.cnorm2[cid]; }
-                    s_hgb[r] = gb; s_hn[r] = nv; s_hcn[r] = cn;
-                }
-            }
-            __syncthreads();
-            LSTAMP(2);
-            auto head_info = [&](uint32_t r, float& g_add, float& g_err, uint32_t& gb, uint32_t& nvec) {
-                const uint64_t key = keys[s_head[r]];
-                const float ci = cost_of((uint32_t)(key >> 32));
-                g_add = ci + 1.01f * eps;
-                if (metric == 0) g_err = sqrtf(fmaxf(g_add, 0.0f));
-                else g_err = sqrtf(fmaxf(qc.qnorm2 + s_hcn[r] + 2.0f * ci + 4.0f * eps, 0.0f));
-                gb = s_hgb[r]; nvec = s_hn[r];
-            };
-            const uint32_t nb0 = (s_hn[0] + 31u) >> 5, nb1 = (s_hn[1] + 31u) >> 5, nb2 = (s_hn[2] + 31u) >> 5, nb3 = (s_hn[3] + 31u) >> 5;
-            static_assert(kSelHead == 4, "four head lists");
-            const uint32_t tot = nb0 + nb1 + nb2 + nb3;
-            const uint32_t ncand = tot < (uint32_t)kThreads ? tot : (uint32_t)kThreads;
-            float myU = INFINITY;
-            uint32_t myN = 0;
-            if (tid < ncand) {
-                uint32_t r = 0, b = tid;
-                if (b >= nb0) { b -= nb0; r = 1; if (b >= nb1) { b -= nb1; r = 2; if (b >= nb2) { b -= nb2; r = 3; } } }
-                float g_add, g_err; uint32_t gb, nvec;
-                head_info(r, g_add, g_err, gb, nvec);
-                const BlockSummary bs = P.bsum[gb + b];
-                const BlockSummaryEx bx = P.bsumx[gb + b];
-                myU = block_ub(bs, bx, g_add, g_err, qc, D, P.ex_bits, P.slack, V == kVarPortable) + 1e-4f * eps;
-                myN = (b + 1 == ((nvec + 31u) >> 5)) ? nvec - b * 32u : 32u;
-                if (P.head_ub) {
-                    uint32_t* hu = P.head_ub + (size_t)q * kHeadUbRow + 10 + 3 * tid;
-                    hu[0] = gb + b; hu[1] = __float_as_uint(myU); hu[2] = myN;
-                }
-            }
-            float* candU = reinterpret_cast<float*>(part);
-            candU[tid] = myU; hist[tid] = myN;
-            if (tid < h) {
-                float g_add, g_err; uint32_t gb, nvec;
-                head_info(tid, g_add, g_err, gb, nvec);
-                if (P.head_ub) {
-                    uint32_t* hu = P.head_ub + (size_t)q * kHeadUbRow;
-                    hu[2 + 2 * tid] = __float_as_uint(g_add); hu[3 + 2 * tid] = __float_as_uint(g_err);
-                    if (tid == 0) { hu[0] = ncand; hu[1] = h; }
-                }
-                atomicMax(reinterpret_cast<int*>(&s_maxh), total_key(g_add));
-            }
-            __syncthreads();
-            if (tid < ncand && myU < INFINITY) {
-                uint32_t cum = 0;
-#pragma unroll 8
-                for (uint32_t j = 0; j < ncand; ++j) cum += candU[j] <= myU ? hist[j] : 0u;
-                if (cum >= P.top_k) atomicMin(reinterpret_cast<int*>(&s_tub), total_key(myU));
-            }
-            __syncthreads();
+            if (!front) head_bound(h, hp0, hp1, hp2, hp3);
             float T_ub = P.fault_dead_all ? -INFINITY : key_to_float((int32_t)s_tub);
             const float cost_maxh = key_to_float((int32_t)s_maxh);
             bool hx_done = false;
@@ -1229,7 +1352,6 @@
                     }
                     LSTAMP(5);
                     __shared__ uint32_t s_zone[512];
-                    __shared__ unsigned long long s_kept[kSelKeptMax];
                     if (zone_scored) {
                         for (uint32_t w = tid; w < 512; w += kThreads) s_zone[w] = 0u;
                         __syncthreads();
@@ -1307,6 +1429,7 @@
             __syncthreads();
             SSTAMP();
             sort_keys(keys, n, cap2, tid);
+            if (front) m_scan = n;
         }
 #ifdef RBQ_SEL_STAMPS
         else SSTAMP();
diff --git a/rabitq-rs_amd/index.py b/rabitq-rs_amd/index.py
--- a/rabitq-rs_amd/index.py
+++ b/rabitq-rs_amd/index.py
@@ -63,6 +63,8 @@
             getattr(L, n_).argtypes = [vp]
         L.rbq_debug_tie_log_stats.restype = None
         L.rbq_debug_tie_log_stats.argtypes = [vp, vp]
+        L.rbq_debug_select_front_stats.restype = None
+        L.rbq_debug_select_front_stats.argtypes = [vp, vp]
         L.rbq_debug_bounce_copies.restype = C.c_uint64
         L.rbq_debug_bounce_copies.argtypes = []
         L.rbq_index_build_device.restype = C.c_int
@@ -507,6 +509,11 @@
         lib().rbq_debug_tie_log_stats(self._h, out.ctypes.data)
         return dict(zip(("replays", "entries", "heap_ops", "overflows"), (int(v) for v in out)))
 
+    def select_front_stats(self):
+        out = np.zeros(4, np.uint64)
+        lib().rbq_debug_select_front_stats(self._h, out.ctypes.data)
+        return dict(zip(("taken", "fell_back_count", "fell_back_overflow", "fell_back_other"), (int(v) for v in out)))
+
     def rank_fallbacks(self):
         return lib().rbq_debug_rank_fallbacks(self._h)
 
```

Result: slower. 7.197 million (-6.8%).
